# bitlayer-org/tap-stark

Hardware: AMD Instinct MI355X
Metric: trace cells/sec (proofs/sec alongside), 2^20x64 BabyBear trace (higher is better)
Workload: dtype u32

## Files before the change

### tap-stark_amd/csrc/alubench.hip

```cpp
#include "blake3.hpp"
#include "kernels.hpp"
#include "sha256.hpp"

namespace ts {

namespace {

constexpr int BF_ITER = 1024, BF_ILP = 8;
constexpr int B3_ITER = 64;

__global__ void __launch_bounds__(256) k_alu_butterflies(uint32_t* __restrict__ out, uint32_t seed) {
    uint32_t a[BF_ILP], b[BF_ILP];
#pragma unroll
    for (int i = 0; i < BF_ILP; i++) {
        a[i] = (seed + threadIdx.x * 7 + i) % P;
        b[i] = (seed * 3 + threadIdx.x + i) % P;
    }
    const uint32_t w = seed % P;
    for (int it = 0; it < BF_ITER; it++) {
#pragma unroll
        for (int i = 0; i < BF_ILP; i++) {
            const uint32_t x = red2p(a[i]);
            const uint32_t t = mont_mul(b[i], w);
            a[i] = x + t;
            b[i] = x - t + P;
        }
    }
    uint32_t s = 0;
#pragma unroll
    for (int i = 0; i < BF_ILP; i++) s ^= a[i] ^ b[i];
    out[blockIdx.x * blockDim.x + threadIdx.x] = s;
}

__global__ void __launch_bounds__(256) k_alu_blake3(uint32_t* __restrict__ out, uint32_t seed) {
    uint32_t m[16], cv[8];
#pragma unroll
    for (int i = 0; i < 16; i++) m[i] = seed * (i + 1) + threadIdx.x + blockIdx.x * 977;
    for (int it = 0; it < B3_ITER; it++) {
        b3::hash64(m, cv);
#pragma unroll
        for (int i = 0; i < 8; i++) {
            m[i] = cv[i];
            m[8 + i] ^= cv[i];
        }
    }
    uint32_t s = 0;
#pragma unroll
    for (int i = 0; i < 8; i++) s ^= cv[i];
    out[blockIdx.x * blockDim.x + threadIdx.x] = s;
}

constexpr int LDSB_ROUNDS = 256;
template <bool WIDE>
__global__ void __launch_bounds__(256) k_alu_butterflies_lds(uint32_t* __restrict__ out, uint32_t seed) {
    __shared__ uint32_t img[4096 + 128 + 16];
    uint32_t v[16];
#pragma unroll
    for (int i = 0; i < 16; i++) v[i] = (seed + threadIdx.x * 7 + i) % P;
    const uint32_t w = seed % P;
    for (int it = 0; it < LDSB_ROUNDS; it++) {
#pragma unroll
        for (int d = 0; d < 4; d++) {
            const int half = 8 >> d;
#pragma unroll
            for (int q = 0; q < 16; q++)
                if ((q & half) == 0) {
                    const uint32_t x = red2p(v[q]);
                    const uint32_t t = mont_mul(v[q + half], w);
                    v[q] = x + t;
                    v[q + half] = x - t + P;
                }
        }
        if (WIDE) {
            uint4* p4 = reinterpret_cast<uint4*>(img) + threadIdx.x * 4 + (threadIdx.x >> 3);
#pragma unroll
            for (int k = 0; k < 4; k++) p4[k] = make_uint4(v[4 * k], v[4 * k + 1], v[4 * k + 2], v[4 * k + 3]);
            __syncthreads();
            const uint4* r4 = reinterpret_cast<const uint4*>(img) + ((threadIdx.x + 64) & 255) * 4 + (((threadIdx.x + 64) & 255) >> 3);
#pragma unroll
            for (int k = 0; k < 4; k++) {
                const uint4 u = r4[k];
                v[4 * k] = u.x; v[4 * k + 1] = u.y; v[4 * k + 2] = u.z; v[4 * k + 3] = u.w;
            }
        } else {
#pragma unroll
            for (int q = 0; q < 16; q++) {
                const uint32_t i = threadIdx.x + 256u * q;
                img[i + (i >> 5)] = v[q];
            }
            __syncthreads();
#pragma unroll
            for (int q = 0; q < 16; q++) {
                const uint32_t i = 16u * threadIdx.x + q;
                v[q] = img[i + (i >> 5)];
            }
        }
        __syncthreads();
    }
    uint32_t s = 0;
#pragma unroll
    for (int i = 0; i < 16; i++) s ^= v[i];
    out[blockIdx.x * blockDim.x + threadIdx.x] = s;
}

constexpr int SHA_ITER = 32;
__global__ void __launch_bounds__(256) k_alu_sha256(uint32_t* __restrict__ out, uint32_t seed) {
    uint32_t m[16], h[8];
    sha::iv(h);
#pragma unroll
    for (int i = 0; i < 16; i++) m[i] = seed * (i + 1) + threadIdx.x + blockIdx.x * 977;
    for (int it = 0; it < SHA_ITER; it++) {
        sha::compress(h, m);
#pragma unroll
        for (int i = 0; i < 8; i++) m[i] ^= h[i];
    }
    uint32_t s = 0;
#pragma unroll
    for (int i = 0; i < 8; i++) s ^= h[i];
    out[blockIdx.x * blockDim.x + threadIdx.x] = s;
}

}

double alu_ceiling(Context& ctx, int kind) {
    TS_REQUIRE(kind >= 0 && kind <= 4, TS_ERR_INVALID,
               "alu_ceiling: kind is 0 (butterflies), 1 (blake3), 2 (sha256), 3 / 4 (butterflies + LDS round trips)");
    const int blocks = ctx.num_cus * 16, threads = 256, reps = 5;
    DevBuf<uint32_t> out(&ctx, (size_t)blocks * threads);
    hipEvent_t e0, e1;
    TS_HIP(hipEventCreate(&e0));
    TS_HIP(hipEventCreate(&e1));
    auto launch = [&] {
        if (kind == 0)
            hipLaunchKernelGGL(k_alu_butterflies, dim3(blocks), dim3(threads), 0, ctx.stream, out.p, 12345u);
        else if (kind == 1)
            hipLaunchKernelGGL(k_alu_blake3, dim3(blocks), dim3(threads), 0, ctx.stream, out.p, 12345u);
        else if (kind == 3)
            hipLaunchKernelGGL(k_alu_butterflies_lds<false>, dim3(blocks), dim3(threads), 0, ctx.stream, out.p, 12345u);
        else if (kind == 4)
            hipLaunchKernelGGL(k_alu_butterflies_lds<true>, dim3(blocks), dim3(threads), 0, ctx.stream, out.p, 12345u);
        else
            hipLaunchKernelGGL(k_alu_sha256, dim3(blocks), dim3(threads), 0, ctx.stream, out.p, 12345u);
    };
    launch();
    TS_HIP(hipEventRecord(e0, ctx.stream));
    for (int r = 0; r < reps; r++) launch();
    TS_HIP(hipEventRecord(e1, ctx.stream));
    TS_HIP(hipEventSynchronize(e1));
    float ms = 0;
    TS_HIP(hipEventElapsedTime(&ms, e0, e1));
    (void)hipEventDestroy(e0);
    (void)hipEventDestroy(e1);
    const double per = (double)ms / reps * 1e-3;
    const double units = kind == 0 ? (double)BF_ITER * BF_ILP : kind == 1 ? (double)B3_ITER
                         : kind == 2 ? (double)SHA_ITER : (double)LDSB_ROUNDS * 32;
    return units * blocks * threads / per;
}

}
```

### tap-stark_amd/csrc/bb.hpp

```cpp
#pragma once
#include <stdint.h>

#if defined(__HIPCC__)
#include <hip/hip_runtime.h>
#define TS_HD __host__ __device__ __forceinline__
#else
#define TS_HD inline
#endif

namespace ts {

constexpr uint32_t P = 0x78000001u;
constexpr uint32_t P_INV = 0x88000001u;
constexpr uint32_t P_NEG_INV = 0x77ffffffu;
constexpr uint32_t R_MOD_P = 0x0ffffffeu;
constexpr uint32_t R2_MOD_P = 0x45dddde3u;
constexpr uint32_t GENERATOR = 31u;
constexpr uint32_t TWO_ADIC_GEN_27 = 0x1a427a41u;
constexpr uint32_t EF_W = 11u;

TS_HD uint32_t umin32(uint32_t a, uint32_t b) { return a < b ? a : b; }
TS_HD uint32_t add(uint32_t a, uint32_t b) {
    uint32_t s = a + b;
    return umin32(s, s - P);
}
TS_HD uint32_t sub(uint32_t a, uint32_t b) {
    uint32_t d = a - b;
    return umin32(d, d + P);
}
TS_HD uint32_t neg(uint32_t a) { return a ? P - a : 0u; }

TS_HD uint32_t mulhi32(uint32_t a, uint32_t b) {
#if defined(__HIP_DEVICE_COMPILE__)
    return __umulhi(a, b);
#else
    return (uint32_t)(((uint64_t)a * b) >> 32);
#endif
}

TS_HD uint32_t mont_reduce(uint64_t t) {
    uint32_t m = (uint32_t)t * P_NEG_INV;
    uint32_t r = (uint32_t)((t + (uint64_t)m * P) >> 32);
    return umin32(r, r - P);
}
TS_HD uint32_t red2p(uint32_t x) { return umin32(x, x - P); }
TS_HD uint32_t mont_mul_lazy(uint32_t a, uint32_t b) {
    const uint64_t t = (uint64_t)a * b;
    const uint32_t m = (uint32_t)t * P_NEG_INV;
    return (uint32_t)((t + (uint64_t)m * P) >> 32);
}
TS_HD uint32_t mont_mul(uint32_t a, uint32_t b) { return mont_reduce((uint64_t)a * b); }
TS_HD uint32_t to_mont(uint32_t a) { return mont_mul(a, R2_MOD_P); }
TS_HD uint32_t from_mont(uint32_t a) { return mont_reduce((uint64_t)a); }

TS_HD uint32_t mul(uint32_t a, uint32_t b) { return mont_mul(to_mont(a), b); }

TS_HD uint32_t pow_canon(uint32_t a, uint64_t e) {
    uint32_t r = R_MOD_P, am = to_mont(a);
    while (e) {
        if (e & 1) r = mont_mul(r, am);
        am = mont_mul(am, am);
        e >>= 1;
    }
    return from_mont(r);
}
TS_HD uint32_t mont_pow(uint32_t am, uint64_t e) {
    uint32_t r = R_MOD_P;
    while (e) {
        if (e & 1) r = mont_mul(r, am);
        am = mont_mul(am, am);
        e >>= 1;
    }
    return r;
}
TS_HD uint32_t mont_inv(uint32_t a) {
    uint32_t a2 = mont_mul(a, a), a3 = mont_mul(a2, a), a6 = mont_mul(a3, a3);
    uint32_t a7 = mont_mul(a6, a), a14 = mont_mul(a7, a7), a15 = mont_mul(a14, a);
    uint32_t r = a7;
    for (int k = 0; k < 4; k++) r = mont_mul(r, r);
    r = mont_mul(r, a7);
    for (int w = 0; w < 6; w++) {
        for (int k = 0; k < 4; k++) r = mont_mul(r, r);
        r = mont_mul(r, a15);
    }
    return r;
}
TS_HD uint32_t inv_canon(uint32_t a) { return pow_canon(a, P - 2); }
TS_HD uint32_t two_adic_generator(unsigned bits) {
    return pow_canon(TWO_ADIC_GEN_27, 1ull << (27 - bits));
}

struct alignas(16) Ef {
    uint32_t c[4];
};

TS_HD Ef ef_zero() { return Ef{{0, 0, 0, 0}}; }
TS_HD Ef ef_add(Ef a, Ef b) {
    return Ef{{add(a.c[0], b.c[0]), add(a.c[1], b.c[1]), add(a.c[2], b.c[2]), add(a.c[3], b.c[3])}};
}
TS_HD Ef ef_sub(Ef a, Ef b) {
    return Ef{{sub(a.c[0], b.c[0]), sub(a.c[1], b.c[1]), sub(a.c[2], b.c[2]), sub(a.c[3], b.c[3])}};
}
TS_HD Ef ef_neg(Ef a) { return Ef{{neg(a.c[0]), neg(a.c[1]), neg(a.c[2]), neg(a.c[3])}}; }
TS_HD bool ef_eq(Ef a, Ef b) {
    return a.c[0] == b.c[0] && a.c[1] == b.c[1] && a.c[2] == b.c[2] && a.c[3] == b.c[3];
}
TS_HD Ef ef_mul_base(Ef a, uint32_t bm) {
    return Ef{{mont_mul(a.c[0], bm), mont_mul(a.c[1], bm), mont_mul(a.c[2], bm), mont_mul(a.c[3], bm)}};
}
TS_HD uint64_t lazy_mac(uint64_t acc, uint32_t a, uint32_t b) { return acc + (uint64_t)a * b; }
TS_HD uint64_t lazy_fix(uint64_t acc) {
#if defined(__HIP_DEVICE_COMPILE__)
    typedef uint32_t v2u __attribute__((ext_vector_type(2)));
    v2u u = __builtin_bit_cast(v2u, acc);
    u.y = umin32(u.y, u.y - P);
    return __builtin_bit_cast(uint64_t, u);
#else
    uint32_t hi = (uint32_t)(acc >> 32);
    hi = umin32(hi, hi - P);
    return ((uint64_t)hi << 32) | (uint32_t)acc;
#endif
}
TS_HD uint32_t lazy_finish(uint64_t acc) { return mont_reduce(lazy_fix(acc)); }

TS_HD Ef ef_mul(Ef a, Ef b) {
    constexpr uint32_t W_M = (uint32_t)(((uint64_t)EF_W << 32) % P);
    const uint32_t w1 = mont_mul(b.c[1], W_M), w2 = mont_mul(b.c[2], W_M), w3 = mont_mul(b.c[3], W_M);
    const uint32_t a0 = a.c[0], a1 = a.c[1], a2 = a.c[2], a3 = a.c[3];
    const uint64_t r0 = lazy_mac(lazy_mac(lazy_mac(lazy_mac(0, a0, b.c[0]), a1, w3), a2, w2), a3, w1);
    const uint64_t r1 = lazy_mac(lazy_mac(lazy_mac(lazy_mac(0, a0, b.c[1]), a1, b.c[0]), a2, w3), a3, w2);
    const uint64_t r2 = lazy_mac(lazy_mac(lazy_mac(lazy_mac(0, a0, b.c[2]), a1, b.c[1]), a2, b.c[0]), a3, w3);
    const uint64_t r3 = lazy_mac(lazy_mac(lazy_mac(lazy_mac(0, a0, b.c[3]), a1, b.c[2]), a2, b.c[1]), a3, b.c[0]);
    return Ef{{lazy_finish(r0), lazy_finish(r1), lazy_finish(r2), lazy_finish(r3)}};
}
TS_HD Ef ef_to_mont(Ef a) { return Ef{{to_mont(a.c[0]), to_mont(a.c[1]), to_mont(a.c[2]), to_mont(a.c[3])}}; }
TS_HD Ef ef_from_mont(Ef a) {
    return Ef{{from_mont(a.c[0]), from_mont(a.c[1]), from_mont(a.c[2]), from_mont(a.c[3])}};
}
TS_HD Ef ef_one_mont() { return Ef{{R_MOD_P, 0, 0, 0}}; }
TS_HD Ef ef_from_base(uint32_t a) { return Ef{{a, 0, 0, 0}}; }

TS_HD void ef_inv_parts(Ef a, Ef& num, uint32_t& nrm) {
    constexpr uint32_t W_M = (uint32_t)(((uint64_t)EF_W << 32) % P);
    uint32_t a0 = a.c[0], a1 = a.c[1], a2 = a.c[2], a3 = a.c[3];
    uint32_t A2_0 = add(mont_mul(a0, a0), mont_mul(W_M, mont_mul(a2, a2)));
    uint32_t A2_1 = mont_mul(add(a0, a0), a2);
    uint32_t B2_0 = add(mont_mul(a1, a1), mont_mul(W_M, mont_mul(a3, a3)));
    uint32_t B2_1 = mont_mul(add(a1, a1), a3);
    uint32_t c0 = sub(A2_0, mont_mul(W_M, B2_1));
    uint32_t c1 = sub(A2_1, B2_0);
    nrm = sub(mont_mul(c0, c0), mont_mul(W_M, mont_mul(c1, c1)));
    Ef conj = Ef{{a0, neg(a1), a2, neg(a3)}};
    Ef cc = Ef{{c0, 0, neg(c1), 0}};
    num = ef_mul(conj, cc);
}
TS_HD Ef ef_inv(Ef a) {
    Ef num;
    uint32_t nrm;
    ef_inv_parts(a, num, nrm);
    return ef_mul_base(num, mont_inv(nrm));
}
TS_HD Ef ef_pow(Ef am, uint64_t e) {
    Ef r = ef_one_mont();
    while (e) {
        if (e & 1) r = ef_mul(r, am);
        am = ef_mul(am, am);
        e >>= 1;
    }
    return r;
}

TS_HD uint32_t bitrev32(uint32_t x, unsigned bits) {
#if defined(__HIP_DEVICE_COMPILE__)
    return bits ? (__brev(x) >> (32 - bits)) : 0u;
#else
    uint32_t r = 0;
    for (unsigned i = 0; i < bits; i++) r |= ((x >> i) & 1u) << (bits - 1 - i);
    return r;
#endif
}

}
```

### tap-stark_amd/csrc/context.cpp

```cpp
#include <errno.h>
#include <stdio.h>
#include <time.h>
#include <stdlib.h>
#include "context.hpp"

#include <string.h>

#include "kernels.hpp"

namespace ts {

static bool poison_knob(uint32_t* word) {
    const char* e = getenv("TS_POOL_POISON");
    if (!e || !*e) return false;
    char* end = nullptr;
    errno = 0;
    const unsigned long v = strtoul(e, &end, 0);
    TS_REQUIRE(errno == 0 && end != e && *end == 0 && e[0] != '-' && v <= 0xFFFFFFFFul, TS_ERR_INVALID,
               "TS_POOL_POISON is not a 32-bit word (decimal, 0x hex or 0 octal)");
    *word = (uint32_t)v;
    return true;
}

Context::Context(int dev) : device(dev) {
    pool_debug = getenv("TS_POOL_DEBUG") != nullptr;
    poison_on = poison_knob(&poison_word);
    int count = 0;
    hipError_t e = hipGetDeviceCount(&count);
    if (e != hipSuccess || count == 0)
        throw Error(TS_ERR_HIP, "no HIP device available: the tap-stark HIP path has no CPU fallback");
    TS_REQUIRE(dev >= 0 && dev < count, TS_ERR_INVALID, "device index out of range");
    TS_HIP(hipSetDevice(dev));
    hipDeviceProp_t prop;
    TS_HIP(hipGetDeviceProperties(&prop, dev));
    num_cus = prop.multiProcessorCount;
    max_lds_per_block = prop.sharedMemPerBlock;
    arch_name = prop.gcnArchName;
    arch_name = arch_name.substr(0, arch_name.find(':'));
    TS_HIP(hipStreamCreateWithFlags(&stream, hipStreamNonBlocking));
}

Context::~Context() {
    (void)hipSetDevice(device);
    if (stream) (void)hipStreamSynchronize(stream);
    if (d_twiddle_fwd) (void)hipFree(d_twiddle_fwd);
    if (d_twiddle_inv) (void)hipFree(d_twiddle_inv);
    for (auto& t : scale_tables) (void)hipFree(t.d);
    for (auto& t : sel_tables)
        if (t.d) (void)hipFree(t.d);
    if (d_ticket) (void)hipFree(d_ticket);
    for (auto& kv : free_blocks) (void)hipFree(kv.second);
    for (auto& kv : live_blocks) (void)hipFree(kv.first);
    if (h_pinned) (void)hipHostFree(h_pinned);
    if (h_mailbox) (void)hipHostFree(h_mailbox);
    if (h_mailbox_big) (void)hipHostFree(h_mailbox_big);
    if (h_arena) (void)hipHostFree(h_arena);
    if (stream) (void)hipStreamDestroy(stream);
}

static size_t round_block(size_t bytes) {
    if (bytes < 512) return 512;
    if (bytes < (1u << 20)) {
        size_t r = 512;
        while (r < bytes) r <<= 1;
        return r;
    }
    const size_t g = 1u << 20;
    return (bytes + g - 1) / g * g;
}

void* Context::alloc(size_t bytes) {
    const size_t sz = round_block(bytes);
    auto it = free_blocks.find(sz);
    void* p = nullptr;
    if (it != free_blocks.end()) {
        p = it->second;
        free_blocks.erase(it);
    } else {
        TS_HIP(hipSetDevice(device));
        if (pool_debug) {
            struct timespec ts_;
            clock_gettime(CLOCK_MONOTONIC, &ts_);
            fprintf(stderr, "[ts pool %p t=%.3f ms] hipMalloc %zu KiB (reserved %zu MiB)\n", (void*)this,
                    ts_.tv_sec * 1e3 + ts_.tv_nsec * 1e-6, sz >> 10, bytes_reserved >> 20);
        }
        hipError_t e = hipMalloc(&p, sz);
        if (e != hipSuccess) {
            release_cache();
            e = hipMalloc(&p, sz);
        }
        if (e != hipSuccess) {
            (void)hipGetLastError();
            throw Error(TS_ERR_OOM, "device allocation failed");
        }
        bytes_reserved += sz;
    }
    live_blocks[p] = sz;
    if (poison_on) poison(p, sz);
    return p;
}

void Context::poison(void* p, size_t bytes) {
    TS_HIP(hipSetDevice(device));
    TS_HIP(hipMemsetD32Async((hipDeviceptr_t)p, (int)poison_word, bytes / 4, stream));
    TS_HIP(hipStreamSynchronize(stream));
    poison_fills++;
}

void Context::free(void* p) {
    if (!p) return;
    auto it = live_blocks.find(p);
    if (it == live_blocks.end()) return;
    free_blocks.emplace(it->second, p);
    live_blocks.erase(it);
}

void Context::release_cache() {
    if (stream) (void)hipStreamSynchronize(stream);
    for (auto& kv : free_blocks) {
        (void)hipFree(kv.second);
        bytes_reserved -= kv.first;
    }
    free_blocks.clear();
}

uint32_t* Context::ticket() {
    if (!d_ticket) {
        TS_HIP(hipMalloc((void**)&d_ticket, 64 * 17));
        TS_HIP(hipMemsetAsync(d_ticket, 0, 64 * 17, stream));
    }
    return d_ticket;
}

const void* Context::stage(const void* src, size_t bytes) {
    const size_t need = (bytes + 63) & ~(size_t)63;
    if (need > h_arena_bytes / 2) {
        sync();
        if (h_arena) (void)hipHostFree(h_arena);
        h_arena = nullptr;
        size_t sz = 1 << 20;
        while (sz / 2 < need) sz <<= 1;
        TS_HIP(hipHostMalloc((void**)&h_arena, sz, hipHostMallocDefault));
        h_arena_bytes = sz;
        h_arena_off = 0;
    }
    if (h_arena_off + need > h_arena_bytes) {
        sync();
        h_arena_off = 0;
    }
    void* p = h_arena + h_arena_off;
    memcpy(p, src, bytes);
    h_arena_off += need;
    return p;
}

void Context::sync_point(void* host, size_t bytes) {
    if (replay_mode == 2 && replay_pos < replay_log.size() && replay_log[replay_pos].size() == bytes) {
        memcpy(host, replay_log[replay_pos++].data(), bytes);
        return;
    }
    sync();
    if (replay_mode == 1) replay_log.emplace_back((const char*)host, (const char*)host + bytes);
}
void Context::d2h_point(void* host_dst, const void* dev_src, size_t bytes) {
    if (replay_mode == 2 && replay_pos < replay_log.size() && replay_log[replay_pos].size() == bytes) {
        memcpy(host_dst, replay_log[replay_pos++].data(), bytes);
        return;
    }
    if (bytes) TS_HIP(hipMemcpyAsync(host_dst, dev_src, bytes, hipMemcpyDeviceToHost, stream));
    sync();
    if (replay_mode == 1) replay_log.emplace_back((const char*)host_dst, (const char*)host_dst + bytes);
}

uint32_t* Context::mailbox(size_t words) {
    constexpr size_t WORDS = 16384;
    if (words > WORDS / 4) {
        if (words > h_mailbox_big_words) {
            sync();
            if (h_mailbox_big) (void)hipHostFree(h_mailbox_big);
            h_mailbox_big = nullptr;
            h_mailbox_big_words = 0;
            TS_HIP(hipHostMalloc((void**)&h_mailbox_big, words * 4, hipHostMallocDefault));
            h_mailbox_big_words = words;
        }
        return h_mailbox_big;
    }
    if (!h_mailbox) TS_HIP(hipHostMalloc((void**)&h_mailbox, WORDS * 4, hipHostMallocDefault));
    const size_t need = (words + 15) & ~(size_t)15;
    if (mailbox_off + need > WORDS) mailbox_off = 0;
    uint32_t* p = h_mailbox + mailbox_off;
    mailbox_off += need;
    return p;
}

void* Context::pinned(size_t bytes) {
    if (bytes > h_pinned_bytes) {
        if (h_pinned) {
            sync();
            (void)hipHostFree(h_pinned);
        }
        size_t sz = 1 << 16;
        while (sz < bytes) sz <<= 1;
        TS_HIP(hipHostMalloc(&h_pinned, sz, hipHostMallocDefault));
        h_pinned_bytes = sz;
    }
    return h_pinned;
}

std::map<std::string, std::pair<uint64_t, double>> Context::take_kernel_timings() {
    std::map<std::string, std::pair<uint64_t, double>> out;
    sync();
    for (auto& ev : kernel_events) {
        float ms = 0;
        (void)hipEventElapsedTime(&ms, ev.e0, ev.e1);
        auto& slot = out[ev.name];
        slot.first += 1;
        slot.second += ms;
        (void)hipEventDestroy(ev.e0);
        (void)hipEventDestroy(ev.e1);
    }
    kernel_events.clear();
    return out;
}

void Context::ensure_twiddles(unsigned log_size) {
    if (log_size <= twiddle_log && d_twiddle_fwd) return;
    TS_REQUIRE(log_size <= 27, TS_ERR_INVALID, "two-adicity of BabyBear is 27");
    sync();
    if (d_twiddle_fwd) (void)hipFree(d_twiddle_fwd);
    if (d_twiddle_inv) (void)hipFree(d_twiddle_inv);
    d_twiddle_fwd = d_twiddle_inv = nullptr;
    const size_t n = (size_t)1 << log_size;
    TS_HIP(hipMalloc((void**)&d_twiddle_fwd, n * 4));
    TS_HIP(hipMalloc((void**)&d_twiddle_inv, n * 4));
    if (poison_on) {
        poison(d_twiddle_fwd, n * 4);
        poison(d_twiddle_inv, n * 4);
    }
    twiddle_log = log_size;
    launch_build_twiddles(*this, d_twiddle_fwd, d_twiddle_inv, log_size);
}

}
```

### tap-stark_amd/csrc/context.hpp

```cpp
#pragma once
#include <hip/hip_runtime.h>
#include <stdint.h>

#include <map>
#include <stdexcept>
#include <string>
#include <vector>

#include "bb.hpp"

namespace ts {

struct Error : std::runtime_error {
    int code;
    Error(int c, const std::string& m) : std::runtime_error(m), code(c) {}
};

struct FinalPolyNotConstant : Error {
    explicit FinalPolyNotConstant(const std::string& m) : Error(5 , m) {}
};

enum : int {
    TS_OK = 0,
    TS_ERR_INVALID = 1,
    TS_ERR_HIP = 2,
    TS_ERR_OOM = 3,
    TS_ERR_UNSUPPORTED = 4,
    TS_ERR_INVARIANT = 5,
    TS_ERR_BUFFER = 6,
    TS_ERR_COMM = 7,
};

#define TS_HIP(expr)                                                                        \
    do {                                                                                    \
        hipError_t _e = (expr);                                                             \
        if (_e != hipSuccess)                                                               \
            throw ts::Error(ts::TS_ERR_HIP, std::string(#expr) + ": " + hipGetErrorString(_e)); \
    } while (0)

#define TS_REQUIRE(cond, code, msg)                   \
    do {                                              \
        if (!(cond)) throw ts::Error((code), (msg));  \
    } while (0)

struct Context {
    int device = 0;
    hipStream_t stream = nullptr;
    std::string last_error;
    int num_cus = 256;
    size_t max_lds_per_block = 64 * 1024;
    std::string arch_name;

    std::multimap<size_t, void*> free_blocks;
    std::map<void*, size_t> live_blocks;
    size_t bytes_reserved = 0;
    bool pool_debug = false;
    bool poison_on = false;
    uint32_t poison_word = 0;
    uint64_t poison_fills = 0;
    void poison(void* p, size_t bytes);

    uint32_t* d_twiddle_fwd = nullptr;
    uint32_t* d_twiddle_inv = nullptr;
    unsigned twiddle_log = 0;

    struct ScaleTable {
        unsigned log_n, log_blowup;
        uint32_t shift;
        uint32_t* d;
        size_t words;
        uint64_t last_use;
    };
    std::vector<ScaleTable> scale_tables;
    uint64_t scale_clock = 0;
    struct SelTable {
        uint32_t* d = nullptr;
        unsigned log_n = ~0u, log_qd = ~0u;
        uint32_t shift = 0;
        uint64_t last_use = 0;
    };
    SelTable sel_tables[2];
    uint64_t sel_clock = 0;

    uint32_t* d_ticket = nullptr;
    uint32_t* ticket();

    unsigned lde_pass_mask = 7;

    uint32_t* h_mailbox = nullptr;
    size_t mailbox_off = 0;
    uint32_t* h_mailbox_big = nullptr;
    size_t h_mailbox_big_words = 0;
    uint32_t* mailbox(size_t words);

    void* h_pinned = nullptr;
    size_t h_pinned_bytes = 0;
    char* h_arena = nullptr;
    size_t h_arena_bytes = 0, h_arena_off = 0;
    const void* stage(const void* src, size_t bytes);

    bool timing = false;
    std::vector<std::pair<std::string, float>> stage_ms;

    struct KernelEvent {
        const char* name;
        hipEvent_t e0, e1;
    };
    bool kernel_timing = false;
    std::vector<KernelEvent> kernel_events;
    std::map<std::string, std::pair<uint64_t, double>> take_kernel_timings();

    uint64_t pow_hints_accepted = 0, pow_hints_rejected = 0, pow_host_grinds = 0;
    uint64_t local_quotient_fallbacks = 0;

    explicit Context(int dev);
    ~Context();
    Context(const Context&) = delete;

    void* alloc(size_t bytes);
    void free(void* p);
    template <class T>
    T* alloc_n(size_t n) { return static_cast<T*>(alloc(n * sizeof(T))); }
    void release_cache();

    int replay_mode = 0;
    size_t replay_pos = 0;
    std::vector<std::vector<char>> replay_log;
    void sync_point(void* host, size_t bytes);
    void d2h_point(void* host_dst, const void* dev_src, size_t bytes);
    void* pinned(size_t bytes);
    void ensure_twiddles(unsigned log_size);
    void sync() { TS_HIP(hipStreamSynchronize(stream)); }
};

template <class T>
struct DevBuf {
    Context* ctx = nullptr;
    T* p = nullptr;
    size_t n = 0;
    DevBuf() = default;
    DevBuf(Context* c, size_t count) : ctx(c), p(c->alloc_n<T>(count)), n(count) {}
    DevBuf(const DevBuf&) = delete;
    DevBuf& operator=(const DevBuf&) = delete;
    DevBuf(DevBuf&& o) noexcept : ctx(o.ctx), p(o.p), n(o.n) { o.p = nullptr; }
    DevBuf& operator=(DevBuf&& o) noexcept {
        if (this != &o) {
            reset();
            ctx = o.ctx; p = o.p; n = o.n; o.p = nullptr;
        }
        return *this;
    }
    ~DevBuf() { reset(); }
    void reset() {
        if (p) ctx->free(p);
        p = nullptr;
    }
};

struct KernelTimer {
    Context* ctx;
    Context::KernelEvent ev;
    bool on;
    KernelTimer(Context* c, const char* name) : ctx(c), on(c->kernel_timing) {
        if (on) {
            ev.name = name;
            (void)hipEventCreate(&ev.e0);
            (void)hipEventCreate(&ev.e1);
            (void)hipEventRecord(ev.e0, ctx->stream);
        }
    }
    ~KernelTimer() {
        if (on) {
            (void)hipEventRecord(ev.e1, ctx->stream);
            ctx->kernel_events.push_back(ev);
        }
    }
};

#define TS_LAUNCH_NAMED(ctx, name, kernel, grid, block, lds, ...)                   \
    do {                                                                            \
        ts::KernelTimer _kt(&(ctx), name);                                          \
        hipLaunchKernelGGL(kernel, grid, block, lds, (ctx).stream, __VA_ARGS__);    \
    } while (0)
#define TS_LAUNCH(ctx, kernel, ...) TS_LAUNCH_NAMED(ctx, #kernel, kernel, __VA_ARGS__)

struct StageTimer {
    Context* ctx;
    const char* name;
    hipEvent_t e0 = nullptr, e1 = nullptr;
    StageTimer(Context* c, const char* n) : ctx(c), name(n) {
        if (ctx->timing) {
            (void)hipEventCreate(&e0);
            (void)hipEventCreate(&e1);
            (void)hipEventRecord(e0, ctx->stream);
        }
    }
    ~StageTimer() {
        if (ctx->timing && e0) {
            (void)hipEventRecord(e1, ctx->stream);
            (void)hipEventSynchronize(e1);
            float ms = 0;
            (void)hipEventElapsedTime(&ms, e0, e1);
            ctx->stage_ms.emplace_back(name, ms);
            (void)hipEventDestroy(e0);
            (void)hipEventDestroy(e1);
        }
    }
};

}
```

### tap-stark_amd/csrc/kernels.hpp

```cpp
#pragma once
#include <stdint.h>

#include "bb.hpp"
#include "context.hpp"
#include "ntt_plan.hpp"

namespace ts {

struct ColMat {
    uint32_t* d = nullptr;
    uint64_t height = 0;
    uint32_t width = 0;
    uint64_t col_stride = 0;
};

void launch_build_twiddles(Context& ctx, uint32_t* W, uint32_t* Winv, unsigned log_size);
void launch_build_shift_tables(Context& ctx, uint32_t* lo, uint32_t* hi, uint32_t n_hi,
                               uint32_t n_cosets, uint32_t shift_mont, unsigned log_N,
                               unsigned log_blowup, uint32_t scale_mont);
const uint32_t* coset_scale_table(Context& ctx, unsigned log_n, unsigned log_blowup, uint32_t shift);
void launch_transpose_bitrev(Context& ctx, const uint32_t* src, uint32_t* dst, unsigned log_n,
                             uint32_t w, uint64_t dst_col_stride, uint32_t src_width = 0);
bool launch_transpose_bitrev_r16(Context& ctx, const uint32_t* src, uint32_t* dst, unsigned log_n, uint32_t w,
                                 uint64_t dst_col_stride, uint32_t src_width = 0);
void launch_transpose_plain(Context& ctx, const uint32_t* src, uint32_t* dst, uint64_t n, uint32_t w,
                            uint64_t dst_col_stride);
void launch_transpose_to_row_major(Context& ctx, const uint32_t* src, uint64_t col_stride,
                                   uint32_t* dst, uint64_t h, uint32_t w);
void launch_transpose_unbitrev(Context& ctx, const uint32_t* src, uint64_t col_stride, uint32_t* dst,
                               unsigned log_h, uint32_t w);
void coset_lde(Context& ctx, uint32_t* evals, uint64_t in_col_stride, uint32_t ncols, unsigned log_n,
               unsigned log_blowup, uint32_t shift, uint32_t* out, uint64_t out_col_stride,
               uint32_t beta0 = 0, uint32_t n_beta = 0, bool first_round_done = false,
               uint32_t* evals2 = nullptr, uint32_t shift2 = 0, uint32_t gw = 0, bool stage_timers = true);

constexpr uint32_t LDE_NO_OWN = 0xffffffffu;
int lde_own_coset_used(unsigned log_n, unsigned log_blowup, uint32_t shift);

inline void ntt_require_shape(const NttPlan& p, uint32_t ncols, uint64_t stride_a, uint64_t stride_b, bool lde) {
    if (const char* why = ntt_plan_refusal(p, ncols, stride_a, stride_b, lde)) throw Error(TS_ERR_INVALID, why);
}
void launch_contig_inverse(Context& ctx, const NttPlan& p, uint32_t* data, uint64_t col_stride, uint32_t ncols,
                           bool first_round_done = false, uint32_t* data2 = nullptr, uint32_t gw = 0xffffffffu);
void launch_contig_forward(Context& ctx, const NttPlan& p, uint32_t* data, uint64_t col_stride, uint32_t ncols,
                           uint32_t n_blocks, uint32_t gw = 0xffffffffu, uint32_t own_a = LDE_NO_OWN,
                           uint32_t own_b = LDE_NO_OWN);

void dft_columns(Context& ctx, uint32_t* cols, uint64_t col_stride, uint32_t ncols, unsigned log_n, bool inverse,
                 uint32_t shift);
void dft_batch(Context& ctx, const uint32_t* in, uint32_t* out, unsigned log_n, uint32_t w, bool inverse,
               uint32_t shift);
void coset_lde_batch(Context& ctx, const uint32_t* in, uint32_t* out, unsigned log_n, uint32_t w, unsigned added_bits,
                     uint32_t shift, bool bit_reversed);
void launch_bit_reverse_rows(Context& ctx, const uint32_t* src, uint32_t* dst, unsigned log_h, uint32_t w);

constexpr int MAX_BATCH_MATS = 64;
struct LeafMats {
    const uint32_t* d[MAX_BATCH_MATS];
    uint64_t col_stride[MAX_BATCH_MATS];
    uint32_t width[MAX_BATCH_MATS];
    uint8_t row_shift[MAX_BATCH_MATS];
    uint32_t n_mats;
    uint32_t total_width;
    const uint32_t* const* cols;
};
void launch_leaf_hash(Context& ctx, const LeafMats& mats, uint64_t height, uint32_t* digests);
void launch_leaf_hash_ef_pairs(Context& ctx, const uint32_t* vec, uint64_t n_rows, uint32_t* digests);
struct DevChallenger;
bool launch_merkle_levels(Context& ctx, uint32_t* tree, unsigned log_leaves,
                          DevChallenger* ch = nullptr, uint32_t* root_out = nullptr,
                          Ef* beta_out = nullptr);
void launch_merkle_tree_from(Context& ctx, uint32_t* tree, unsigned log_leaves, unsigned first_level,
                             DevChallenger* ch, uint32_t* root_out, Ef* beta_out);
bool leaf_tree_enabled(unsigned log_leaves);
void launch_commit_tree(Context& ctx, const LeafMats& mats, unsigned log_leaves, uint32_t* tree,
                        uint32_t* root_out = nullptr);
void launch_shard_top(Context& ctx, const uint32_t* subroots, uint32_t G, uint32_t* top,
                      DevChallenger* ch, uint32_t* root_out, Ef* beta_out);
void launch_merkle_one_level(Context& ctx, const uint32_t* children, uint32_t* parents,
                             uint64_t n_parents);
void launch_merkle_inject(Context& ctx, uint32_t* nodes, const uint32_t* inj, uint64_t n);
inline uint64_t merkle_level_offset(unsigned log_leaves, unsigned level) {
    uint64_t off = 0;
    for (unsigned l = 0; l < level; l++) off += (uint64_t)1 << (log_leaves - l);
    return off;
}
inline uint64_t merkle_total_digests(unsigned log_leaves) { return ((uint64_t)2 << log_leaves) - 1; }

struct AirProgram;
const uint32_t* selector_table(Context& ctx, unsigned log_n, unsigned log_qd, uint32_t shift);
constexpr int MAX_QUOTIENT_CHUNKS = 64;
struct QuotOut {
    uint32_t* chunk[MAX_QUOTIENT_CHUNKS];
};
void launch_quotient(Context& ctx, const AirProgram& air, const ColMat& trace_lde, unsigned log_n,
                     unsigned log_qd, const uint32_t* d_consts_mont, const uint32_t* d_alpha_pows_mont,
                     const QuotOut& out, uint64_t row_begin = 0, uint64_t row_end = 0,
                     uint32_t shift = GENERATOR, const ColMat* prep_lde = nullptr, const ColMat* aux_lde = nullptr);
void launch_chunk_mix(Context& ctx, uint32_t* const* d_chunk_ptrs, uint32_t qd, uint64_t rows, uint64_t col_stride,
                      const uint32_t* d_mix_mont);

void launch_check_constraints(Context& ctx, const AirProgram& air, const uint32_t* trace_row_major,
                              uint64_t n, const uint32_t* d_consts_mont,
                              unsigned long long* d_violation, const uint32_t* prep_row_major = nullptr,
                              const uint32_t* aux_row_major = nullptr);

void launch_bary_weights(Context& ctx, unsigned log_n, const Ef* points_mont, uint32_t n_points,
                         Ef* out, uint32_t coset_gen = 0);
struct BaryPending {
    DevBuf<uint32_t> partial[4];
    uint32_t* out[4] = {nullptr, nullptr, nullptr, nullptr};
    uint32_t n_blocks[4] = {0, 0, 0, 0}, n_words[4] = {0, 0, 0, 0};
    uint32_t n = 0, capacity = 2;
};
void launch_bary_dots(Context& ctx, const ColMat& m, unsigned log_n, const Ef* weights,
                      uint32_t n_points, Ef* out, BaryPending* pending = nullptr);
void launch_bary_finish(Context& ctx, BaryPending& pending);
struct ReduceArgs {
    Ef z_mont[2];
    Ef off_mont[2];
    Ef rys[2];
    uint32_t n_points;
    uint32_t accumulate;
};
void launch_reduce(Context& ctx, const ColMat& m, unsigned log_h, const uint32_t* d_alpha_pows_mont,
                   const ReduceArgs& args, Ef* ro);
struct FusedReduceArgs {
    Ef z_mont[2];
    Ef off_t[2];
    Ef k0, k1;
    const uint32_t* chunk_w;
    const uint32_t* chunk[MAX_QUOTIENT_CHUNKS];
    uint64_t chunk_stride;
    uint32_t n_chunks;
    uint64_t row0, rows;
};
void launch_reduce_fused(Context& ctx, const ColMat& trace, unsigned log_h,
                         const uint32_t* d_alpha_pows_mont, const FusedReduceArgs& args, Ef* ro,
                         const ColMat* prep = nullptr, const Ef* prep_off_mont = nullptr,
                         const ColMat* aux = nullptr, const Ef* aux_off_mont = nullptr);
void launch_reduce_low(Context& ctx, const ColMat& trace, unsigned log_n, const uint32_t* d_alpha_pows_mont,
                       const FusedReduceArgs& args, const Ef* weights, uint32_t* out);
void launch_ef_interleave(Context& ctx, const uint32_t* cols, uint64_t col_stride, uint64_t rows, Ef* out);

void launch_fri_fold(Context& ctx, const Ef* in, uint64_t h, Ef beta_canonical, Ef* out,
                     uint32_t* next_digests);
void launch_fri_fold_dev(Context& ctx, const Ef* in, uint64_t h, const Ef* d_beta, Ef* out,
                         uint32_t* next_digests, uint64_t h_global = 0, uint64_t row0 = 0);
struct FriRoundLaunch {
    const Ef* prev = nullptr;
    const Ef* d_beta_prev = nullptr;
    Ef* cur = nullptr;
    uint64_t h = 0;
    uint32_t* tree = nullptr;
    DevChallenger* ch = nullptr;
    uint32_t* root_out = nullptr;
    Ef* beta_out = nullptr;
    uint64_t h_global = 0, row0 = 0;
};
void launch_fri_commit_round(Context& ctx, const FriRoundLaunch& r);
constexpr int FRI_TAIL_LOG = 10;
constexpr uint32_t FRI_POW_NONE = 0xffffffffu;
void launch_fri_tail(Context& ctx, const Ef* in, uint32_t L0, uint32_t blowup, DevChallenger* ch,
                     Ef* tail_vecs, uint32_t* tail_trees, uint32_t* roots_out, Ef* betas_out,
                     Ef* final_out, uint32_t pow_bits = 0, uint32_t* pow_out = nullptr,
                     const Ef* beta_in = nullptr);
void launch_vec_add(Context& ctx, Ef* acc, const Ef* other, uint64_t n);
struct FriGatherDesc {
    const uint32_t* vec;
    const uint32_t* tree;
    uint32_t log_leaves;
    uint32_t shift;
    uint64_t out_vals;
    uint64_t out_path;
};
struct RowGatherJob {
    LeafMats mats;
    uint32_t shift;
    uint32_t pad;
    uint64_t out;
};
void launch_gather_queries(Context& ctx, const RowGatherJob* d_rows, uint32_t n_rows, uint32_t max_row_width,
                           const FriGatherDesc* d_descs, uint32_t n_descs, uint32_t max_log_leaves,
                           const uint32_t* d_indices, uint32_t n_idx, uint32_t* out);

double alu_ceiling(Context& ctx, int kind);
double bench_stage(Context& ctx, int stage, unsigned log_n, uint32_t width, unsigned log_blowup, uint32_t reps);

void launch_trace_fibonacci(Context& ctx, uint32_t* out, uint32_t a, uint32_t b, uint64_t n);
void launch_trace_synth_mul(Context& ctx, uint32_t* out, uint64_t n, uint32_t width, uint64_t seed);
void launch_trace_synth_ext(Context& ctx, uint32_t* out, uint64_t n, uint32_t width, uint64_t seed);

enum : uint8_t { COL_U32 = 0, COL_U16 = 1, COL_U8 = 2, COL_MONTY32 = 3, COL_MONTY31 = 4 };
struct IngestPlan {
    bool planar = false;
    uint64_t height = 0;
    uint32_t width = 0;
    uint64_t stride = 0;
    uint64_t bytes = 0;
    int uniform4 = -1;
    std::vector<uint64_t> table;
};
IngestPlan ingest_plan(const uint8_t* kinds, uint32_t n_kinds, bool planar, uint64_t row_stride, uint64_t height,
                       uint32_t width);
void launch_ingest(Context& ctx, const IngestPlan& plan, const uint8_t* src, uint32_t* out);
void launch_scale_words(Context& ctx, const uint32_t* in, uint32_t* out, uint64_t n, uint32_t mult);
uint32_t monty_ingest_factor(uint32_t kind);

}
```

### tap-stark_amd/csrc/ntt.hip

```cpp
#include "kernels.hpp"

namespace ts {

constexpr int SHIFT_LO_BITS = 10;

__global__ void k_build_twiddles(uint32_t* __restrict__ W, uint32_t* __restrict__ Winv,
                                 unsigned log_size) {
    uint32_t idx = blockIdx.x * blockDim.x + threadIdx.x;
    if (idx >= (1u << log_size)) return;
    if (idx == 0) {
        W[0] = R_MOD_P;
        Winv[0] = R_MOD_P;
        return;
    }
    unsigned logm = 31 - __clz(idx);
    uint32_t i = idx - (1u << logm);
    uint32_t g27 = to_mont(TWO_ADIC_GEN_27);
    uint32_t g = mont_pow(g27, 1ull << (27 - (logm + 1)));
    uint32_t e = bitrev32(i, logm);
    uint32_t w = mont_pow(g, e);
    W[idx] = w;
    Winv[idx] = mont_inv(w);
}

void launch_build_twiddles(Context& ctx, uint32_t* W, uint32_t* Winv, unsigned log_size) {
    uint32_t n = 1u << log_size;
    TS_LAUNCH(ctx, k_build_twiddles, dim3((n + 255) / 256), dim3(256), 0, W, Winv, log_size);
    TS_HIP(hipGetLastError());
}

__global__ void k_build_shift_tables(uint32_t* __restrict__ lo, uint32_t* __restrict__ hi,
                                     uint32_t n_hi, uint32_t shift_mont, unsigned log_N,
                                     unsigned log_blowup, uint32_t scale_mont) {
    uint32_t beta = blockIdx.y;
    uint32_t j = blockIdx.x * blockDim.x + threadIdx.x;
    uint32_t n_lo = 1u << SHIFT_LO_BITS;
    if (j >= n_lo + n_hi) return;
    uint32_t g27 = to_mont(TWO_ADIC_GEN_27);
    uint32_t gN = mont_pow(g27, 1ull << (27 - log_N));
    uint32_t s = mont_mul(shift_mont, mont_pow(gN, bitrev32(beta, log_blowup)));
    if (j < n_lo) {
        lo[beta * n_lo + j] = mont_mul(mont_pow(s, j), scale_mont);
    } else {
        uint32_t jj = j - n_lo;
        hi[beta * n_hi + jj] = mont_pow(s, (uint64_t)jj << SHIFT_LO_BITS);
    }
}

void launch_build_shift_tables(Context& ctx, uint32_t* lo, uint32_t* hi, uint32_t n_hi,
                               uint32_t n_cosets, uint32_t shift_mont, unsigned log_N,
                               unsigned log_blowup, uint32_t scale_mont) {
    const uint32_t n_lo = 1u << SHIFT_LO_BITS;
    TS_LAUNCH(ctx, k_build_shift_tables, dim3((n_lo + n_hi + 255) / 256, n_cosets), dim3(256), 0, lo,
              hi, n_hi, shift_mont, log_N, log_blowup, scale_mont);
    TS_HIP(hipGetLastError());
}

__global__ void __launch_bounds__(256)
k_build_scale_table(const uint32_t* __restrict__ lo, const uint32_t* __restrict__ hi, uint32_t n_hi,
                    unsigned log_n, uint32_t* __restrict__ T) {
    const uint32_t beta = blockIdx.y;
    const uint64_t k = (uint64_t)blockIdx.x * blockDim.x + threadIdx.x;
    if (k >= (1ull << log_n)) return;
    const uint32_t n_lo = 1u << SHIFT_LO_BITS;
    T[((uint64_t)beta << log_n) + k] =
        mont_mul(lo[beta * n_lo + (k & (n_lo - 1))], hi[(uint64_t)beta * n_hi + (k >> SHIFT_LO_BITS)]);
}

const uint32_t* coset_scale_table(Context& ctx, unsigned log_n, unsigned log_blowup, uint32_t shift) {
    for (auto& t : ctx.scale_tables)
        if (t.log_n == log_n && t.log_blowup == log_blowup && t.shift == shift) {
            t.last_use = ++ctx.scale_clock;
            return t.d;
        }
    const uint32_t n_cosets = 1u << log_blowup;
    const size_t words = (size_t)n_cosets << log_n;
    size_t total = words * 4;
    for (auto& t : ctx.scale_tables) total += t.words * 4;
    while (!ctx.scale_tables.empty() && (ctx.scale_tables.size() >= 8 || total > (2ull << 30))) {
        size_t victim = 0;
        for (size_t i = 1; i < ctx.scale_tables.size(); i++)
            if (ctx.scale_tables[i].last_use < ctx.scale_tables[victim].last_use) victim = i;
        ctx.sync();
        total -= ctx.scale_tables[victim].words * 4;
        (void)hipFree(ctx.scale_tables[victim].d);
        ctx.scale_tables.erase(ctx.scale_tables.begin() + victim);
    }
    uint32_t* d = nullptr;
    TS_HIP(hipMalloc((void**)&d, words * 4));
    if (ctx.poison_on) ctx.poison(d, words * 4);
    const uint64_t n = 1ull << log_n;
    const uint32_t n_lo = 1u << SHIFT_LO_BITS;
    const uint32_t n_hi = log_n > (unsigned)SHIFT_LO_BITS ? 1u << (log_n - SHIFT_LO_BITS) : 1u;
    DevBuf<uint32_t> lo(&ctx, (size_t)n_cosets * n_lo), hi(&ctx, (size_t)n_cosets * n_hi);
    const uint32_t n_inv_mont = to_mont(inv_canon((uint32_t)(n % P)));
    launch_build_shift_tables(ctx, lo.p, hi.p, n_hi, n_cosets, to_mont(shift), log_n + log_blowup, log_blowup,
                              n_inv_mont);
    TS_LAUNCH(ctx, k_build_scale_table, dim3((unsigned)((n + 255) / 256), n_cosets), dim3(256), 0,
              (const uint32_t*)lo.p, (const uint32_t*)hi.p, n_hi, log_n, d);
    TS_HIP(hipGetLastError());
    ctx.scale_tables.push_back(Context::ScaleTable{log_n, log_blowup, shift, d, words, ++ctx.scale_clock});
    return d;
}

template <bool TO_COLUMNS, bool BITREV>
__global__ void __launch_bounds__(256)
k_transpose_tile(const uint32_t* __restrict__ src, uint32_t* __restrict__ dst, uint64_t h, unsigned log_h,
                 uint32_t w, uint64_t col_stride, uint32_t rm_width) {
    __shared__ uint32_t tile[64][65];
    const uint64_t p0 = (uint64_t)blockIdx.x * 64;
    const uint32_t c0 = blockIdx.y * 64;
    const uint32_t tx = threadIdx.x & 63, ty = threadIdx.x >> 6;
    auto row_of = [&](uint64_t p) -> uint64_t { return BITREV ? bitrev32((uint32_t)p, log_h) : p; };
    if (p0 + 64 <= h && c0 + 64 <= w) {
        const uint64_t rm = row_of(p0) * rm_width + c0 + tx;
        const uint64_t rm_step = BITREV ? (uint64_t)rm_width << (log_h - 6) : rm_width;
        const uint64_t cm = (uint64_t)(c0 + ty) * col_stride + p0 + tx;
        auto rm_at = [&](int k) {
            const uint32_t i = ty + 4 * (uint32_t)k;
            return rm + (uint64_t)(BITREV ? __brev(i) >> 26 : i) * rm_step;
        };
        auto cm_at = [&](int k) { return cm + (uint64_t)(4 * k) * col_stride; };
        uint32_t t[16];
#pragma unroll
        for (int k = 0; k < 16; k++) t[k] = src[TO_COLUMNS ? rm_at(k) : cm_at(k)];
#pragma unroll
        for (int k = 0; k < 16; k++) (TO_COLUMNS ? tile[ty + 4 * k][tx] : tile[tx][ty + 4 * k]) = t[k];
        __syncthreads();
#pragma unroll
        for (int k = 0; k < 16; k++) t[k] = TO_COLUMNS ? tile[tx][ty + 4 * k] : tile[ty + 4 * k][tx];
#pragma unroll
        for (int k = 0; k < 16; k++) dst[TO_COLUMNS ? cm_at(k) : rm_at(k)] = t[k];
        return;
    }
    auto rm_ok = [&](uint32_t j) { return p0 + j < h && c0 + tx < w; };
    auto cm_ok = [&](uint32_t j) { return c0 + j < w && p0 + tx < h; };
    auto rm_at = [&](uint32_t j) { return row_of(p0 + j) * rm_width + c0 + tx; };
    auto cm_at = [&](uint32_t j) { return (uint64_t)(c0 + j) * col_stride + p0 + tx; };
#pragma unroll
    for (int k = 0; k < 16; k++) {
        const uint32_t j = ty + 4 * (uint32_t)k;
        if (TO_COLUMNS ? rm_ok(j) : cm_ok(j)) (TO_COLUMNS ? tile[j][tx] : tile[tx][j]) = src[TO_COLUMNS ? rm_at(j) : cm_at(j)];
    }
    __syncthreads();
#pragma unroll
    for (int k = 0; k < 16; k++) {
        const uint32_t j = ty + 4 * (uint32_t)k;
        if (TO_COLUMNS ? cm_ok(j) : rm_ok(j)) dst[TO_COLUMNS ? cm_at(j) : rm_at(j)] = TO_COLUMNS ? tile[tx][j] : tile[j][tx];
    }
}

template <bool TO_COLUMNS, bool BITREV>
static void launch_transpose_tile(Context& ctx, const char* name, const uint32_t* src, uint32_t* dst, uint64_t h,
                                  unsigned log_h, uint32_t w, uint64_t col_stride, uint32_t rm_width) {
    if (w == 0 || h == 0) return;
    TS_LAUNCH_NAMED(ctx, name, (k_transpose_tile<TO_COLUMNS, BITREV>), dim3((unsigned)((h + 63) / 64), (w + 63) / 64),
                    dim3(256), 0, src, dst, h, log_h, w, col_stride, rm_width);
    TS_HIP(hipGetLastError());
}

void launch_transpose_bitrev(Context& ctx, const uint32_t* src, uint32_t* dst, unsigned log_n,
                             uint32_t w, uint64_t dst_col_stride, uint32_t src_width) {
    launch_transpose_tile<true, true>(ctx, "k_transpose_bitrev", src, dst, 1ull << log_n, log_n, w, dst_col_stride,
                                      src_width ? src_width : w);
}

void launch_transpose_plain(Context& ctx, const uint32_t* src, uint32_t* dst, uint64_t n, uint32_t w,
                            uint64_t dst_col_stride) {
    launch_transpose_tile<true, false>(ctx, "k_transpose_plain", src, dst, n, 0, w, dst_col_stride, w);
}

void launch_transpose_to_row_major(Context& ctx, const uint32_t* src, uint64_t col_stride,
                                   uint32_t* dst, uint64_t h, uint32_t w) {
    launch_transpose_tile<false, false>(ctx, "k_transpose_to_row_major", src, dst, h, 0, w, col_stride, w);
}

void launch_transpose_unbitrev(Context& ctx, const uint32_t* src, uint64_t col_stride, uint32_t* dst,
                               unsigned log_h, uint32_t w) {
    launch_transpose_tile<false, true>(ctx, "k_transpose_unbitrev", src, dst, 1ull << log_h, log_h, w, col_stride, w);
}

}
```

### tap-stark_amd/csrc/ntt_dft.hip

```cpp
#include <algorithm>

#include "ntt_rounds.hpp"

namespace ts {

constexpr int DFT_LO_BITS = 10;

__device__ __forceinline__ uint32_t dft_factor(const uint32_t* __restrict__ lo, const uint32_t* __restrict__ hi,
                                               uint32_t k) {
    return mont_mul(lo[k & ((1u << DFT_LO_BITS) - 1)], hi[k >> DFT_LO_BITS]);
}

template <bool INV, bool SCALE, int PLAN, int TILE = TILE_ELEMS, int NTM = NT_MID>
__global__ void __launch_bounds__(NTM)
k_dft_mid(uint32_t* data, uint64_t col_stride, unsigned log_len, unsigned log_T, unsigned row_shift,
          const uint32_t* __restrict__ W, const uint32_t* __restrict__ f_lo, const uint32_t* __restrict__ f_hi) {
    __shared__ uint32_t s[padded(TILE)];
    constexpr int PER_THREAD = TILE / NTM;
    if (PLAN == 1) {
        log_len = 8;
        log_T = 5;
    }
    const uint32_t j2_0 = blockIdx.x << log_T;
    uint32_t* g = data + (uint64_t)blockIdx.y * col_stride + j2_0;
    const uint32_t total = 1u << (log_len + log_T);
    const uint32_t tmask = (1u << log_T) - 1;
    auto off = [&](uint32_t i) { return ((i >> log_T) << row_shift) + (i & tmask); };
    if constexpr (PLAN == 1) {
        uint32_t t[PER_THREAD];
#pragma unroll
        for (int k = 0; k < PER_THREAD; k++) t[k] = g[off(threadIdx.x + (uint32_t)k * NTM)];
#pragma unroll
        for (int k = 0; k < PER_THREAD; k++) {
            const uint32_t i = threadIdx.x + (uint32_t)k * NTM;
            if (!INV && SCALE) t[k] = mont_mul_lazy(t[k], dft_factor(f_lo, f_hi, off(i) + j2_0));
            s[pad(i)] = t[k];
        }
    } else {
        for (uint32_t i = threadIdx.x; i < total; i += NTM) {
            uint32_t v = g[off(i)];
            if (!INV && SCALE) v = mont_mul_lazy(v, dft_factor(f_lo, f_hi, off(i) + j2_0));
            s[pad(i)] = v;
        }
    }
    __syncthreads();
    if constexpr (PLAN == 1) {
        if (!INV) {
            radix_round<4, false, 9, NTM, true>(s, 13, 0, 0, 0, W);
            radix_round<4, false, 5, NTM>(s, 13, 4, 0, 0, W);
        } else {
            radix_round<4, true, 5, NTM>(s, 13, 4, 0, 0, W);
            radix_round<4, true, 9, NTM, true>(s, 13, 0, 0, 0, W);
        }
    } else {
        if (!INV) tile_forward_rt<NTM>(s, log_len, log_T, 0, 0, W);
        else tile_inverse_rt<NTM>(s, log_len, log_T, 0, 0, W);
    }
    auto finish = [&](uint32_t v, uint32_t i) {
        if (INV) return SCALE ? mont_mul(v, dft_factor(f_lo, f_hi, off(i) + j2_0)) : red2p(v);
        return row_shift != 0 ? v : red2p(v);
    };
    if constexpr (PLAN == 1) {
        uint32_t t[PER_THREAD];
#pragma unroll
        for (int k = 0; k < PER_THREAD; k++) t[k] = s[pad(threadIdx.x + (uint32_t)k * NTM)];
#pragma unroll
        for (int k = 0; k < PER_THREAD; k++) {
            const uint32_t i = threadIdx.x + (uint32_t)k * NTM;
            g[off(i)] = finish(t[k], i);
        }
    } else {
        for (uint32_t i = threadIdx.x; i < total; i += NTM) g[off(i)] = finish(s[pad(i)], i);
    }
}

__global__ void __launch_bounds__(256)
k_bit_reverse_rows(const uint32_t* __restrict__ src, uint32_t* __restrict__ dst, unsigned log_h, uint32_t w) {
    const uint64_t idx = ((uint64_t)blockIdx.y * gridDim.x + blockIdx.x) * 256 + threadIdx.x;
    const uint64_t r = idx / w;
    if (r >> log_h) return;
    const uint32_t c = (uint32_t)(idx - r * w);
    dst[idx] = src[(uint64_t)bitrev32((uint32_t)r, log_h) * w + c];
}

void launch_bit_reverse_rows(Context& ctx, const uint32_t* src, uint32_t* dst, unsigned log_h, uint32_t w) {
    const uint64_t blocks = ((((uint64_t)w) << log_h) + 255) / 256;
    const uint32_t gx = (uint32_t)std::min<uint64_t>(blocks, 1u << 20);
    TS_LAUNCH(ctx, k_bit_reverse_rows, dim3(gx, (uint32_t)((blocks + gx - 1) / gx)), dim3(256), 0, src, dst, log_h, w);
    TS_HIP(hipGetLastError());
}

template <bool INV, bool SCALE>
static void launch_dft_mid_of(Context& ctx, const NttPlan& p, uint32_t* cols, uint64_t col_stride, uint32_t ncols,
                              const uint32_t* f_lo, const uint32_t* f_hi, const char* const (&names)[3]) {
    const uint32_t* W = INV ? ctx.d_twiddle_inv : ctx.d_twiddle_fwd;
    auto launch = [&](auto kernel) {
        TS_LAUNCH_NAMED(ctx, names[(int)p.mid], kernel, dim3(p.tiles, ncols), dim3(NT_MID), 0, cols, col_stride,
                        p.log_len, p.log_T, p.row_shift, W, f_lo, f_hi);
    };
    if (p.mid == NttMid::TILE16384) launch(k_dft_mid<INV, SCALE, 0, 16384>);
    else if (p.mid == NttMid::FIXED256) launch(k_dft_mid<INV, SCALE, 1>);
    else launch(k_dft_mid<INV, SCALE, 0>);
}

static void launch_dft_mid(Context& ctx, const NttPlan& p, uint32_t* cols, uint64_t col_stride, uint32_t ncols,
                           bool inverse, bool scale, const uint32_t* f_lo, const uint32_t* f_hi) {
    if (inverse)
        launch_dft_mid_of<true, true>(ctx, p, cols, col_stride, ncols, f_lo, f_hi,
                                      {"(k_dft_mid<true, true, 0>)", "(k_dft_mid<true, true, 1>)",
                                       "(k_dft_mid<true, true, 0, 16384>)"});
    else if (scale)
        launch_dft_mid_of<false, true>(ctx, p, cols, col_stride, ncols, f_lo, f_hi,
                                       {"(k_dft_mid<false, true, 0>)", "(k_dft_mid<false, true, 1>)",
                                        "(k_dft_mid<false, true, 0, 16384>)"});
    else
        launch_dft_mid_of<false, false>(ctx, p, cols, col_stride, ncols, f_lo, f_hi,
                                        {"(k_dft_mid<false, false, 0>)", "(k_dft_mid<false, false, 1>)",
                                         "(k_dft_mid<false, false, 0, 16384>)"});
}

void dft_columns(Context& ctx, uint32_t* cols, uint64_t col_stride, uint32_t ncols, unsigned log_n, bool inverse,
                 uint32_t shift) {
    if (ncols == 0) return;
    TS_REQUIRE(shift != 0 && shift < P, TS_ERR_INVALID, "dft: the coset shift must be in [1, p)");
    const NttPlan p = ntt_plan(log_n);
    ntt_require_shape(p, ncols, col_stride, 0, false);
    ctx.ensure_twiddles(log_n == 0 ? 1 : log_n);

    const bool scale = inverse || shift != 1;
    DevBuf<uint32_t> lo, hi;
    if (scale) {
        const uint32_t n_hi = log_n > (unsigned)DFT_LO_BITS ? 1u << (log_n - DFT_LO_BITS) : 1u;
        lo = DevBuf<uint32_t>(&ctx, 1u << DFT_LO_BITS);
        hi = DevBuf<uint32_t>(&ctx, n_hi);
        const uint32_t n_inv = inv_canon((uint32_t)((1ull << log_n) % P));
        launch_build_shift_tables(ctx, lo.p, hi.p, n_hi, 1, to_mont(inverse ? inv_canon(shift) : shift), log_n, 0,
                                  inverse ? to_mont(n_inv) : R_MOD_P);
    }
    if (inverse) {
        if (p.two_pass) launch_contig_inverse(ctx, p, cols, col_stride, ncols);
        launch_dft_mid(ctx, p, cols, col_stride, ncols, true, true, lo.p, hi.p);
    } else {
        launch_dft_mid(ctx, p, cols, col_stride, ncols, false, scale, lo.p, hi.p);
        if (p.two_pass) launch_contig_forward(ctx, p, cols, col_stride, ncols, 1);
    }
    TS_HIP(hipGetLastError());
}

void dft_batch(Context& ctx, const uint32_t* in, uint32_t* out, unsigned log_n, uint32_t w, bool inverse,
               uint32_t shift) {
    const uint64_t n = 1ull << log_n;
    DevBuf<uint32_t> cols(&ctx, (size_t)w * n);
    if (inverse) {
        launch_transpose_bitrev(ctx, in, cols.p, log_n, w, n);
        dft_columns(ctx, cols.p, n, w, log_n, true, shift);
        launch_transpose_to_row_major(ctx, cols.p, n, out, n, w);
    } else {
        launch_transpose_plain(ctx, in, cols.p, n, w, n);
        dft_columns(ctx, cols.p, n, w, log_n, false, shift);
        launch_transpose_unbitrev(ctx, cols.p, n, out, log_n, w);
    }
}

void coset_lde_batch(Context& ctx, const uint32_t* in, uint32_t* out, unsigned log_n, uint32_t w, unsigned added_bits,
                     uint32_t shift, bool bit_reversed) {
    const uint64_t n = 1ull << log_n, N = n << added_bits;
    DevBuf<uint32_t> cols(&ctx, (size_t)w * n), lde(&ctx, (size_t)w * N);
    const bool r16 = lde_own_coset_used(log_n, added_bits, shift) < 0 &&
                     launch_transpose_bitrev_r16(ctx, in, cols.p, log_n, w, n);
    if (!r16) launch_transpose_bitrev(ctx, in, cols.p, log_n, w, n);
    coset_lde(ctx, cols.p, n, w, log_n, added_bits, shift, lde.p, N, 0, 0, r16);
    if (bit_reversed) launch_transpose_to_row_major(ctx, lde.p, N, out, N, w);
    else launch_transpose_unbitrev(ctx, lde.p, N, out, log_n + added_bits, w);
}

}
```

### tap-stark_amd/csrc/ntt_lde.hip

```cpp
#include <stdlib.h>

#include <optional>
#include <type_traits>

#include "ntt_rounds.hpp"

namespace ts {

template <int LM, bool SKIP_R16 = false>
__global__ void __launch_bounds__(chunk_threads(LM))
k_intt_contig(uint32_t* __restrict__ data, uint64_t col_stride, unsigned log_n,
              const uint32_t* __restrict__ Winv, uint32_t* __restrict__ data2, uint32_t gw) {
    __shared__ uint32_t s[padded(1 << LM)];
    const uint32_t c = blockIdx.x;
    uint32_t* col = blockIdx.y < gw ? data + (uint64_t)blockIdx.y * col_stride
                                    : data2 + (uint64_t)(blockIdx.y - gw) * col_stride;
    uint32_t* g = col + ((uint64_t)c << LM);
    chunk_load<LM>(s, g);
    chunk_rounds<LM, true, SKIP_R16>(s, log_n - LM, c, Winv);
    chunk_store<LM, false>(s, g);
}

__global__ void __launch_bounds__(256)
k_transpose_bitrev_r16(const uint32_t* __restrict__ src, uint32_t* __restrict__ dst, unsigned log_n,
                       uint32_t w, uint64_t dst_col_stride, uint32_t src_width,
                       const uint32_t* __restrict__ Winv) {
    __shared__ uint32_t tile[64][65];
    const uint32_t p0 = blockIdx.x << 6;
    const uint32_t c0 = blockIdx.y * 64;
    const uint32_t tx = threadIdx.x & 63, ty = threadIdx.x >> 6;
    const uint32_t rb = bitrev32(p0, log_n);
    const uint64_t row_step = (uint64_t)src_width << (log_n - 6);
    uint32_t v[16];
    if (c0 + tx < w) {
        const uint32_t* sp = src + (uint64_t)rb * src_width + c0 + tx;
#pragma unroll
        for (int q = 0; q < 16; q++) v[q] = sp[(uint64_t)(__brev(16 * ty + (uint32_t)q) >> 26) * row_step];
    } else {
#pragma unroll
        for (int q = 0; q < 16; q++) v[q] = 0;
    }
    radix_butterflies<4, true, false>(v, log_n - 4, 0, 0, (p0 >> 4) + ty, Winv);
#pragma unroll
    for (int q = 0; q < 16; q++) tile[16 * ty + q][tx] = v[q];
    __syncthreads();
    uint32_t t[16];
#pragma unroll
    for (int k = 0; k < 16; k++) t[k] = tile[tx][ty + 4 * k];
    uint32_t* dp = dst + (uint64_t)(c0 + ty) * dst_col_stride + p0 + tx;
#pragma unroll
    for (int k = 0; k < 16; k++)
        if (c0 + ty + 4 * k < w) dp[(uint64_t)(4 * k) * dst_col_stride] = t[k];
}

template <int LM, int CPW>
__device__ __forceinline__ void lde_fwd_contig_block(uint32_t* __restrict__ out, uint64_t out_col_stride, unsigned log_n,
                                                     const uint32_t* __restrict__ W, const uint32_t beta) {
    __shared__ uint32_t s[padded(1 << LM)];
    constexpr int NT = chunk_threads(LM);
    constexpr int NV = (1 << LM) / 4 / NT;
    uint32_t* col = out + (uint64_t)blockIdx.y * out_col_stride + ((uint64_t)beta << log_n);
    if constexpr (CPW == 1) {
        const uint32_t c = blockIdx.x;
        uint32_t* o = col + ((uint64_t)c << LM);
        chunk_load<LM>(s, o);
        chunk_rounds<LM, false>(s, log_n - LM, c, W);
        chunk_store<LM, true>(s, o);
    } else {
        const uint32_t c0 = blockIdx.x * CPW;
        uint4 v[NV];
        {
            const uint4* g4 = reinterpret_cast<const uint4*>(col + ((uint64_t)c0 << LM));
#pragma unroll
            for (int k = 0; k < NV; k++) v[k] = g4[threadIdx.x + (uint32_t)k * NT];
        }
#pragma unroll 1
        for (int i = 0; i < CPW; i++) {
            const uint32_t c = c0 + i;
#pragma unroll
            for (int k = 0; k < NV; k++) {
                const uint32_t i4 = threadIdx.x + (uint32_t)k * NT;
                const uint32_t a = 4 * i4 + (i4 >> 3);
                s[a] = v[k].x;
                s[a + 1] = v[k].y;
                s[a + 2] = v[k].z;
                s[a + 3] = v[k].w;
            }
            __syncthreads();
            if (i + 1 < CPW) {
                const uint4* g4 = reinterpret_cast<const uint4*>(col + ((uint64_t)(c + 1) << LM));
#pragma unroll
                for (int k = 0; k < NV; k++) v[k] = g4[threadIdx.x + (uint32_t)k * NT];
            }
            chunk_rounds<LM, false>(s, log_n - LM, c, W);
            chunk_store<LM, true>(s, col + ((uint64_t)c << LM));
            __syncthreads();
        }
    }
}

template <int LM, int CPW = 1>
__global__ void __launch_bounds__(chunk_threads(LM), CPW > 1 ? 4 : 1)
k_lde_fwd_contig(uint32_t* __restrict__ out, uint64_t out_col_stride, unsigned log_n,
                 const uint32_t* __restrict__ W) {
    lde_fwd_contig_block<LM, CPW>(out, out_col_stride, log_n, W, blockIdx.z);
}

template <int LM, int CPW = 1>
__global__ void __launch_bounds__(chunk_threads(LM), CPW > 1 ? 4 : 1)
k_lde_fwd_contig_own(uint32_t* __restrict__ out, uint64_t out_col_stride, unsigned log_n,
                     const uint32_t* __restrict__ W, uint32_t gw, uint32_t own_a, uint32_t own_b) {
    const uint32_t own = blockIdx.y < gw ? own_a : own_b;
    lde_fwd_contig_block<LM, CPW>(out, out_col_stride, log_n, W, blockIdx.z + (blockIdx.z >= own ? 1u : 0u));
}

template <int PLAN, int TILE = TILE_ELEMS, int NTM = NT_MID, int LM = LOG_M, bool OWN = false>
__global__ void __launch_bounds__(NTM)
k_lde_mid(const uint32_t* __restrict__ evals, uint64_t in_col_stride, uint32_t* __restrict__ out,
          uint64_t out_col_stride, unsigned log_n, unsigned log_len, unsigned log_T,
          unsigned row_shift, unsigned beta0, unsigned n_cosets, const uint32_t* __restrict__ W,
          const uint32_t* __restrict__ Winv, const uint32_t* __restrict__ scale_a,
          const uint32_t* __restrict__ evals2, const uint32_t* __restrict__ scale_b, uint32_t gw,
          uint32_t own_a, uint32_t own_b) {
    __shared__ uint32_t s[padded(TILE)];
    constexpr int PER_THREAD = TILE / NTM;
    if (PLAN == 1) {
        log_len = 8;
        log_T = 5;
    }
    const bool remap = PLAN == 0 && log_T < 5 && gridDim.x >= 8;
    uint32_t bx = remap ? (blockIdx.x & 7) * (gridDim.x >> 3) + (blockIdx.x >> 3) : blockIdx.x;
    uint32_t col_id = blockIdx.y;
    if constexpr (PLAN == 1) {
        const uint32_t ncols = gridDim.x >> (LM - 5);
        bx = (blockIdx.x & 31) + 32 * (blockIdx.x / (32 * ncols));
        col_id = (blockIdx.x >> 5) % ncols;
    }
    const uint32_t j2_0 = bx << log_T;
    const uint32_t* g = (col_id < gw ? evals + (uint64_t)col_id * in_col_stride
                                     : evals2 + (uint64_t)(col_id - gw) * in_col_stride) + j2_0;
    const uint32_t* __restrict__ scale = col_id < gw ? scale_a : scale_b;
    const uint32_t own = OWN ? (col_id < gw ? own_a : own_b) : 0xffffffffu;
    const uint32_t total = 1u << (log_len + log_T);
    const uint32_t tmask = (1u << log_T) - 1;
    if constexpr (PLAN == 1) {
        uint32_t t[PER_THREAD];
#pragma unroll
        for (int k = 0; k < PER_THREAD; k++) {
            const uint32_t i = threadIdx.x + (uint32_t)k * NTM;
            t[k] = g[((uint64_t)(i >> log_T) << row_shift) + (i & tmask)];
        }
#pragma unroll
        for (int k = 0; k < PER_THREAD; k++) s[pad(threadIdx.x + (uint32_t)k * NTM)] = t[k];
    } else {
        for (uint32_t i = threadIdx.x; i < total; i += NTM)
            s[pad(i)] = g[((uint64_t)(i >> log_T) << row_shift) + (i & tmask)];
    }
    __syncthreads();
    if (PLAN == 1) {
        radix_round<4, true, 5, NTM>(s, 13, 4, 0, 0, Winv);
    } else {
        tile_inverse_rt<NTM>(s, log_len, log_T, 0, 0, Winv);
    }
    uint32_t coef[PER_THREAD];
#pragma unroll
    for (int k = 0; k < PER_THREAD; k++) {
        const uint32_t i = threadIdx.x + (uint32_t)k * NTM;
        coef[k] = i < total ? s[pad(i)] : 0u;
    }
    constexpr int GP = PER_THREAD / 16;
    if constexpr (PLAN == 1) {
#pragma unroll
        for (int j = 0; j < GP; j++) {
            uint32_t v[16];
#pragma unroll
            for (int q = 0; q < 16; q++) v[q] = coef[j + GP * q];
            radix_butterflies<4, true, true>(v, 0, 0, 0, 0, Winv);
#pragma unroll
            for (int q = 0; q < 16; q++) coef[j + GP * q] = v[q];
        }
    }
    constexpr bool PREFETCH = PLAN == 1;
    uint32_t scv[PREFETCH ? 16 : 1];
    const uint32_t* scp = nullptr;
    if constexpr (PREFETCH) {
        const uint32_t i0 = threadIdx.x;
        scp = scale + ((uint64_t)(i0 >> 5) << LM) + (i0 & 31) + j2_0;
        const uint32_t first = OWN && own == 0 ? 1u : 0u;
#pragma unroll
        for (int q = 0; q < 16; q++)
            scv[q] = (scp + ((uint64_t)(beta0 + first) << log_n))[(uint64_t)q * (NTM >> 5) << LM];
    }
    for (uint32_t bl = 0; bl < n_cosets; bl++) {
        if (OWN && bl == own) continue;
        const uint32_t beta = beta0 + bl;
        const uint32_t* sc = scale + ((uint64_t)beta << log_n);
        __syncthreads();
        if constexpr (PLAN == 1) {
#pragma unroll
            for (int j = 0; j < GP; j++) {
                uint32_t v[16];
#pragma unroll
                for (int q = 0; q < 16; q++) v[q] = mont_mul_lazy(coef[j + GP * q], scv[q]);
                const uint32_t nb = OWN && bl + 1 == own ? bl + 2 : bl + 1;
                if (nb < n_cosets) {
                    const uint32_t* nx = scp + ((uint64_t)(beta0 + nb) << log_n);
#pragma unroll
                    for (int q = 0; q < 16; q++) scv[q] = nx[(uint64_t)q * (NTM >> 5) << LM];
                }
                radix_butterflies<4, false, true>(v, 0, 0, 0, 0, W);
#pragma unroll
                for (int q = 0; q < 16; q++) s[pad(threadIdx.x + (uint32_t)(j + GP * q) * NTM)] = v[q];
            }
            __syncthreads();
            uint32_t* og = out + (uint64_t)col_id * out_col_stride + ((uint64_t)bl << log_n) + j2_0;
            radix_round<4, false, 5, NTM>(s, 13, 4, 0, 0, W);
            uint32_t t[PER_THREAD];
#pragma unroll
            for (int k = 0; k < PER_THREAD; k++) t[k] = s[pad(threadIdx.x + (uint32_t)k * NTM)];
            uint32_t* ot = og + ((uint64_t)(threadIdx.x >> 5) << LM) + (threadIdx.x & 31);
#pragma unroll
            for (int k = 0; k < PER_THREAD; k++) ot[(uint64_t)k * (NTM >> 5) << LM] = t[k];
            continue;
        } else {
#pragma unroll
            for (int k = 0; k < PER_THREAD; k++) {
                const uint32_t i = threadIdx.x + (uint32_t)k * NTM;
                if (i < total) {
                    const uint32_t kk = ((i >> log_T) << row_shift) + (i & tmask) + j2_0;
                    s[pad(i)] = mont_mul_lazy(coef[k], sc[kk]);
                }
            }
            __syncthreads();
            tile_forward_rt<NTM>(s, log_len, log_T, 0, 0, W);
        }
        uint32_t* o = out + (uint64_t)col_id * out_col_stride + ((uint64_t)bl << log_n) + j2_0;
        if (row_shift != 0) {
            for (uint32_t i = threadIdx.x; i < total; i += NTM)
                o[((uint64_t)(i >> log_T) << row_shift) + (i & tmask)] = s[pad(i)];
        } else {
            for (uint32_t i = threadIdx.x; i < total; i += NTM)
                o[((uint64_t)(i >> log_T) << row_shift) + (i & tmask)] = red2p(s[pad(i)]);
        }
    }
}

template <bool VEC>
__global__ void __launch_bounds__(256)
k_lde_own_copy(const uint32_t* __restrict__ evals, uint64_t in_col_stride, uint32_t* __restrict__ out,
               uint64_t out_col_stride, unsigned log_n, const uint32_t* __restrict__ evals2, uint32_t gw,
               uint32_t own_a, uint32_t own_b) {
    const uint32_t col = blockIdx.y;
    const uint32_t* src = col < gw ? evals + (uint64_t)col * in_col_stride
                                   : evals2 + (uint64_t)(col - gw) * in_col_stride;
    uint32_t* dst = out + (uint64_t)col * out_col_stride + ((uint64_t)(col < gw ? own_a : own_b) << log_n);
    if constexpr (VEC) {
        const uint4* s4 = reinterpret_cast<const uint4*>(src) + (uint64_t)blockIdx.x * 1024 + threadIdx.x;
        uint4* d4 = reinterpret_cast<uint4*>(dst) + (uint64_t)blockIdx.x * 1024 + threadIdx.x;
        uint4 v[4];
#pragma unroll
        for (int k = 0; k < 4; k++) v[k] = s4[256 * k];
#pragma unroll
        for (int k = 0; k < 4; k++) d4[256 * k] = v[k];
    } else {
        const uint64_t i = (uint64_t)blockIdx.x * 256 + threadIdx.x;
        if (i < (1ull << log_n)) dst[i] = src[i];
    }
}

constexpr const char* INTT_NAME[3] = {"k_intt_contig<12>", "k_intt_contig<13>", "k_intt_contig<14>"};
constexpr const char* INTT_R16_NAME[3] = {"(k_intt_contig<12, true>)", "(k_intt_contig<13, true>)",
                                          "(k_intt_contig<14, true>)"};
constexpr const char* FWD_NAME[3] = {"k_lde_fwd_contig<12>", "k_lde_fwd_contig<13>", "(k_lde_fwd_contig<14, 4>)"};

template <class F>
static void with_chunk_log(unsigned LM, F&& f) {
    if (LM == 12) f(std::integral_constant<int, 12>{});
    else if (LM == 13) f(std::integral_constant<int, 13>{});
    else f(std::integral_constant<int, 14>{});
}

bool launch_transpose_bitrev_r16(Context& ctx, const uint32_t* src, uint32_t* dst, unsigned log_n, uint32_t w,
                                 uint64_t dst_col_stride, uint32_t src_width) {
    if (w == 0 || !ntt_plan(log_n).fused_first_round) return false;
    ctx.ensure_twiddles(log_n);
    TS_LAUNCH(ctx, k_transpose_bitrev_r16, dim3(1u << (log_n - 6), (w + 63) / 64), dim3(256), 0, src, dst, log_n, w,
              dst_col_stride, src_width ? src_width : w, (const uint32_t*)ctx.d_twiddle_inv);
    TS_HIP(hipGetLastError());
    return true;
}

void launch_contig_inverse(Context& ctx, const NttPlan& p, uint32_t* data, uint64_t col_stride, uint32_t ncols,
                           bool first_round_done, uint32_t* data2, uint32_t gw) {
    const uint32_t* Winv = ctx.d_twiddle_inv;
    with_chunk_log(p.LM, [&](auto lm) {
        constexpr int LM = decltype(lm)::value;
        const dim3 g(p.chunks, ncols), b(chunk_threads(LM));
        if (first_round_done)
            TS_LAUNCH_NAMED(ctx, INTT_R16_NAME[LM - 12], (k_intt_contig<LM, true>), g, b, 0, data, col_stride, p.log_n,
                            Winv, data2, gw);
        else
            TS_LAUNCH_NAMED(ctx, INTT_NAME[LM - 12], k_intt_contig<LM>, g, b, 0, data, col_stride, p.log_n, Winv, data2,
                            gw);
    });
}

static void launch_lde_mid(Context& ctx, const NttPlan& p, const uint32_t* evals, uint64_t in_col_stride,
                           uint32_t* out, uint64_t out_col_stride, uint32_t ncols, uint32_t beta0, uint32_t n_beta,
                           const uint32_t* scale, const uint32_t* evals2, const uint32_t* scale2, uint32_t gw,
                           uint32_t own_a, uint32_t own_b) {
    const uint32_t *W = ctx.d_twiddle_fwd, *Winv = ctx.d_twiddle_inv;
    const dim3 grid(p.tiles, ncols), b(NT_MID);
    const dim3 grid1(p.tiles * ncols);
#define TS_MID_ARGS \
    evals, in_col_stride, out, out_col_stride, p.log_n, p.log_len, p.log_T, p.row_shift, beta0, n_beta, W, Winv, scale, \
        evals2, scale2, gw, own_a, own_b
    if (own_a != LDE_NO_OWN && p.mid == NttMid::FIXED256 && p.LM == 12)
        TS_LAUNCH_NAMED(ctx, "k_lde_mid<1>", (k_lde_mid<1, TILE_ELEMS, NT_MID, 12, true>), grid1, b, 0, TS_MID_ARGS);
    else if (own_a != LDE_NO_OWN && p.mid == NttMid::FIXED256 && p.LM == 13)
        TS_LAUNCH_NAMED(ctx, "(k_lde_mid<1, 8192, 512, 13>)", (k_lde_mid<1, 8192, 512, 13, true>), grid1, b, 0,
                        TS_MID_ARGS);
    else if (own_a != LDE_NO_OWN && p.mid == NttMid::FIXED256)
        TS_LAUNCH_NAMED(ctx, "(k_lde_mid<1, 8192, 512, 14>)", (k_lde_mid<1, 8192, 512, 14, true>), grid1, b, 0,
                        TS_MID_ARGS);
    else if (own_a != LDE_NO_OWN)
        TS_LAUNCH_NAMED(ctx, "k_lde_mid<0>", (k_lde_mid<0, TILE_ELEMS, NT_MID, LOG_M, true>), grid, b, 0, TS_MID_ARGS);
    else if (p.mid == NttMid::TILE16384)
        TS_LAUNCH_NAMED(ctx, "(k_lde_mid<0, 16384>)", (k_lde_mid<0, 16384>), grid, b, 0, TS_MID_ARGS);
    else if (p.mid == NttMid::FIXED256 && p.LM == 12)
        TS_LAUNCH_NAMED(ctx, "k_lde_mid<1>", k_lde_mid<1>, grid1, b, 0, TS_MID_ARGS);
    else if (p.mid == NttMid::FIXED256 && p.LM == 13)
        TS_LAUNCH_NAMED(ctx, "(k_lde_mid<1, 8192, 512, 13>)", (k_lde_mid<1, 8192, 512, 13>), grid1, b, 0, TS_MID_ARGS);
    else if (p.mid == NttMid::FIXED256)
        TS_LAUNCH_NAMED(ctx, "(k_lde_mid<1, 8192, 512, 14>)", (k_lde_mid<1, 8192, 512, 14>), grid1, b, 0, TS_MID_ARGS);
    else
        TS_LAUNCH_NAMED(ctx, "k_lde_mid<0>", k_lde_mid<0>, grid, b, 0, TS_MID_ARGS);
#undef TS_MID_ARGS
}

void launch_contig_forward(Context& ctx, const NttPlan& p, uint32_t* data, uint64_t col_stride, uint32_t ncols,
                           uint32_t n_blocks, uint32_t gw, uint32_t own_a, uint32_t own_b) {
    const uint32_t* W = ctx.d_twiddle_fwd;
    with_chunk_log(p.LM, [&](auto lm) {
        constexpr int LM = decltype(lm)::value;
        constexpr int CPW = LM == 14 ? 4 : 1;
        if (own_a != LDE_NO_OWN)
            TS_LAUNCH_NAMED(ctx, FWD_NAME[LM - 12], (k_lde_fwd_contig_own<LM, CPW>),
                            dim3(p.chunks / CPW, ncols, n_blocks - 1), dim3(chunk_threads(LM)), 0, data, col_stride,
                            p.log_n, W, gw, own_a, own_b);
        else
            TS_LAUNCH_NAMED(ctx, FWD_NAME[LM - 12], (k_lde_fwd_contig<LM, CPW>), dim3(p.chunks / CPW, ncols, n_blocks),
                            dim3(chunk_threads(LM)), 0, data, col_stride, p.log_n, W);
    });
}

int lde_own_coset_used(unsigned log_n, unsigned log_blowup, uint32_t shift) {
    if (const char* e = getenv("TS_LDE_OWN_COSET"); e && *e && atoi(e) == 0) return -1;
    if (log_blowup == 0 || log_n + log_blowup > 27 || ntt_plan(log_n).mid == NttMid::TILE16384) return -1;
    return lde_own_coset(log_n, log_blowup, shift);
}

void coset_lde(Context& ctx, uint32_t* evals, uint64_t in_col_stride, uint32_t ncols, unsigned log_n,
               unsigned log_blowup, uint32_t shift, uint32_t* out, uint64_t out_col_stride,
               uint32_t beta0, uint32_t n_beta, bool first_round_done, uint32_t* evals2, uint32_t shift2,
               uint32_t gw, bool stage_timers) {
    if (ncols == 0) return;
    TS_REQUIRE(evals2 == nullptr || (gw >= 1 && gw < ncols && shift2 != 0), TS_ERR_INVALID,
               "coset_lde: second matrix needs its first column and its shift");
    if (evals2 == nullptr) gw = 0xffffffffu;
    TS_REQUIRE(log_n + log_blowup <= 27, TS_ERR_INVALID, "coset_lde: log_n + log_blowup > 27");
    const NttPlan p = ntt_plan(log_n);
    ntt_require_shape(p, ncols, in_col_stride, out_col_stride, true);
    TS_REQUIRE(!first_round_done || p.fused_first_round, TS_ERR_INVARIANT,
               "coset_lde: no contiguous inverse pass at this size");
    ctx.ensure_twiddles(log_n == 0 ? 1 : log_n);

    const uint32_t n_cosets = 1u << log_blowup;
    if (n_beta == 0) n_beta = n_cosets - beta0;
    TS_REQUIRE(beta0 < n_cosets && n_beta <= n_cosets - beta0, TS_ERR_INVALID, "coset_lde: coset range");
    const uint32_t* scale = coset_scale_table(ctx, log_n, log_blowup, shift);
    const uint32_t* scale2 = evals2 ? coset_scale_table(ctx, log_n, log_blowup, shift2) : nullptr;

    uint32_t own_a = LDE_NO_OWN, own_b = LDE_NO_OWN;
    if (beta0 == 0 && n_beta == n_cosets && !first_round_done && ctx.lde_pass_mask == 7u) {
        const int a = lde_own_coset_used(log_n, log_blowup, shift);
        const int b = evals2 ? lde_own_coset_used(log_n, log_blowup, shift2) : a;
        if (a >= 0 && b >= 0) {
            own_a = (uint32_t)a;
            own_b = (uint32_t)b;
            const uint64_t n = 1ull << log_n;
            if (p.two_pass)
                TS_LAUNCH_NAMED(ctx, "k_lde_own_copy", k_lde_own_copy<true>, dim3((unsigned)(n >> 12), ncols), dim3(256), 0,
                                (const uint32_t*)evals, in_col_stride, out, out_col_stride, log_n,
                                (const uint32_t*)evals2, gw, own_a, own_b);
            else
                TS_LAUNCH_NAMED(ctx, "k_lde_own_copy", k_lde_own_copy<false>, dim3((unsigned)((n + 255) / 256), ncols),
                                dim3(256), 0, (const uint32_t*)evals, in_col_stride, out, out_col_stride, log_n,
                                (const uint32_t*)evals2, gw, own_a, own_b);
        }
    }

    if (!p.two_pass) {
        launch_lde_mid(ctx, p, evals, in_col_stride, out, out_col_stride, ncols, beta0, n_beta, scale, evals2, scale2,
                       gw, own_a, own_b);
    } else {
        if (ctx.lde_pass_mask & 1u) {
            std::optional<StageTimer> t;
            if (stage_timers) t.emplace(&ctx, "lde: inverse NTT, contiguous stages");
            launch_contig_inverse(ctx, p, evals, in_col_stride, ncols, first_round_done, evals2, gw);
        }
        std::optional<StageTimer> t_rest;
        if (stage_timers) t_rest.emplace(&ctx, "lde: strided pass + forward NTT of the owned cosets");
        if (ctx.lde_pass_mask & 2u)
            launch_lde_mid(ctx, p, evals, in_col_stride, out, out_col_stride, ncols, beta0, n_beta, scale, evals2,
                           scale2, gw, own_a, own_b);
        if (ctx.lde_pass_mask & 4u) launch_contig_forward(ctx, p, out, out_col_stride, ncols, n_beta, gw, own_a, own_b);
    }
    TS_HIP(hipGetLastError());
}

}
```

### tap-stark_amd/csrc/ntt_rounds.hpp

```cpp
#pragma once
#include "kernels.hpp"
#include "ntt_plan.hpp"

namespace ts {

constexpr int NT_MID = 512;
constexpr int chunk_threads(int lm) { return lm == 14 ? 512 : 256; }

__device__ __forceinline__ uint32_t pad(uint32_t i) { return i + (i >> 5); }
constexpr int padded(int n) { return n + (n >> 5); }

template <int K, bool INV, bool TOP>
__device__ __forceinline__ void radix_butterflies(uint32_t (&v)[1 << K], unsigned s_base, unsigned u0,
                                                  uint32_t c, uint32_t hi,
                                                  const uint32_t* __restrict__ W) {
    constexpr int R = 1 << K;
    if (!INV) {
#pragma unroll
        for (int d = 0; d < K; d++) {
            const int half = R >> (d + 1);
            const uint32_t* __restrict__ wp = W + ((1u << (s_base + u0 + d)) + (c << (u0 + d)) + (hi << d));
#pragma unroll
            for (int q = 0; q < R; q++) {
                if ((q & half) == 0) {
                    const uint32_t a = red2p(v[q]);
                    uint32_t t = v[q + half];
                    if (TOP && (q >> (K - d)) == 0) t = red2p(t);
                    else t = mont_mul(t, wp[q >> (K - d)]);
                    v[q] = a + t;
                    v[q + half] = a - t + P;
                }
            }
        }
    } else {
#pragma unroll
        for (int d = K - 1; d >= 0; d--) {
            const int half = R >> (d + 1);
            const uint32_t* __restrict__ wp = W + ((1u << (s_base + u0 + d)) + (c << (u0 + d)) + (hi << d));
#pragma unroll
            for (int q = 0; q < R; q++) {
                if ((q & half) == 0) {
                    const uint32_t a = red2p(v[q]), b = red2p(v[q + half]);
                    v[q] = a + b;
                    uint32_t dlt = a - b + P;
                    if (!(TOP && (q >> (K - d)) == 0)) dlt = mont_mul_lazy(dlt, wp[q >> (K - d)]);
                    v[q + half] = dlt;
                }
            }
        }
    }
}

template <int K, bool INV, int LOG_DL, int NTH, bool TOP = false>
__device__ __forceinline__ void radix_round(uint32_t* s, unsigned log_total, unsigned u0,
                                            unsigned s_base, uint32_t c,
                                            const uint32_t* __restrict__ W) {
    constexpr int R = 1 << K;
    const unsigned log_dl = LOG_DL >= 0 ? (unsigned)LOG_DL : log_total - u0 - K;
    const uint32_t n_groups = 1u << (log_total - K);
    for (uint32_t g0 = threadIdx.x; g0 < n_groups; g0 += NTH) {
        uint32_t g = g0;
        if (LOG_DL == 4 && K < 5) {
            constexpr uint32_t B = 9 - K;
            const uint32_t x = ((g >> 4) ^ (g >> B)) & 1u;
            g ^= (x << 4) | (x << B);
        }
        const uint32_t lo = g & ((1u << log_dl) - 1);
        const uint32_t hi = g >> log_dl;
        const uint32_t base = (hi << (K + log_dl)) + lo;
        const uint32_t pbase = pad(base);
        uint32_t addr[R];
#pragma unroll
        for (int q = 0; q < R; q++) {
            if (LOG_DL >= 5)
                addr[q] = pbase + (uint32_t)q * ((1u << (LOG_DL >= 5 ? LOG_DL : 5)) +
                                                 (1u << (LOG_DL >= 5 ? LOG_DL - 5 : 0)));
            else if (LOG_DL == 4)
                addr[q] = pbase + 16u * (uint32_t)q + ((uint32_t)q >> 1);
            else if (LOG_DL == 0 && K == 4)
                addr[q] = pbase + (uint32_t)q;
            else
                addr[q] = pad(base + ((uint32_t)q << log_dl));
        }
        uint32_t v[R];
#pragma unroll
        for (int q = 0; q < R; q++) v[q] = s[addr[q]];
        radix_butterflies<K, INV, TOP>(v, s_base, u0, c, hi, W);
#pragma unroll
        for (int q = 0; q < R; q++) s[addr[q]] = v[q];
    }
    __syncthreads();
}

template <bool INV, int NTH>
__device__ __forceinline__ void radix_round_rt(int k, uint32_t* s, unsigned log_total, unsigned u0,
                                               unsigned s_base, uint32_t c,
                                               const uint32_t* __restrict__ W) {
    switch (k) {
        case 4: radix_round<4, INV, -1, NTH>(s, log_total, u0, s_base, c, W); break;
        case 3: radix_round<3, INV, -1, NTH>(s, log_total, u0, s_base, c, W); break;
        case 2: radix_round<2, INV, -1, NTH>(s, log_total, u0, s_base, c, W); break;
        default: radix_round<1, INV, -1, NTH>(s, log_total, u0, s_base, c, W); break;
    }
}

template <int NTH>
__device__ __forceinline__ void tile_forward_rt(uint32_t* s, unsigned log_len, unsigned log_T,
                                                unsigned s_base, uint32_t c,
                                                const uint32_t* __restrict__ W) {
    if (log_len == 0) return;
    const unsigned nr = (log_len + 3) / 4, q = log_len / nr, rem = log_len % nr;
    unsigned u = 0;
    for (unsigned r = 0; r < nr; r++) {
        const unsigned k = q + (r < rem ? 1u : 0u);
        radix_round_rt<false, NTH>((int)k, s, log_len + log_T, u, s_base, c, W);
        u += k;
    }
}
template <int NTH>
__device__ __forceinline__ void tile_inverse_rt(uint32_t* s, unsigned log_len, unsigned log_T,
                                                unsigned s_base, uint32_t c,
                                                const uint32_t* __restrict__ Winv) {
    if (log_len == 0) return;
    const unsigned nr = (log_len + 3) / 4, q = log_len / nr, rem = log_len % nr;
    unsigned u = log_len;
    for (int r = (int)nr - 1; r >= 0; r--) {
        const unsigned k = q + ((unsigned)r < rem ? 1u : 0u);
        u -= k;
        radix_round_rt<true, NTH>((int)k, s, log_len + log_T, u, s_base, c, Winv);
    }
}

template <int LM>
__device__ __forceinline__ void chunk_load(uint32_t* s, const uint32_t* __restrict__ g) {
    constexpr int NT = chunk_threads(LM);
    const uint4* g4 = reinterpret_cast<const uint4*>(g);
    uint4 v[(1 << LM) / 4 / NT];
#pragma unroll
    for (int k = 0; k < (1 << LM) / 4 / NT; k++) v[k] = g4[threadIdx.x + (uint32_t)k * NT];
#pragma unroll
    for (int k = 0; k < (1 << LM) / 4 / NT; k++) {
        const uint32_t i4 = threadIdx.x + (uint32_t)k * NT;
        const uint32_t a = 4 * i4 + (i4 >> 3);
        s[a] = v[k].x;
        s[a + 1] = v[k].y;
        s[a + 2] = v[k].z;
        s[a + 3] = v[k].w;
    }
    __syncthreads();
}
template <int LM, bool CANON>
__device__ __forceinline__ void chunk_store(const uint32_t* s, uint32_t* __restrict__ g) {
    constexpr int NT = chunk_threads(LM);
    uint4* g4 = reinterpret_cast<uint4*>(g);
#pragma unroll
    for (int k = 0; k < (1 << LM) / 4 / NT; k++) {
        const uint32_t i4 = threadIdx.x + (uint32_t)k * NT;
        const uint32_t a = 4 * i4 + (i4 >> 3);
        if (CANON)
            g4[i4] = make_uint4(red2p(s[a]), red2p(s[a + 1]), red2p(s[a + 2]), red2p(s[a + 3]));
        else
            g4[i4] = make_uint4(s[a], s[a + 1], s[a + 2], s[a + 3]);
    }
}

template <int LM, bool INV, bool SKIP_R16 = false>
__device__ __forceinline__ void chunk_rounds(uint32_t* s, unsigned sb, uint32_t c, const uint32_t* __restrict__ W) {
    constexpr int NT = chunk_threads(LM);
    constexpr int K0 = LM == 12 ? 4 : 5;
    constexpr int K1 = LM == 14 ? 5 : 4;
    static_assert(K0 + K1 + 4 == LM, "chunk plan");
    if (!INV) {
        radix_round<K0, false, LM - K0, NT>(s, LM, 0, sb, c, W);
        radix_round<K1, false, 4, NT>(s, LM, K0, sb, c, W);
        radix_round<4, false, 0, NT>(s, LM, K0 + K1, sb, c, W);
    } else {
        if (!SKIP_R16) radix_round<4, true, 0, NT>(s, LM, K0 + K1, sb, c, W);
        radix_round<K1, true, 4, NT>(s, LM, K0, sb, c, W);
        radix_round<K0, true, LM - K0, NT>(s, LM, 0, sb, c, W);
    }
}

}
```

### tap-stark_amd/probe/field_probe.hip

```cpp
#include <stdio.h>
#include <string.h>

#include <vector>

#include "bb.hpp"
#include "ntt_rounds.hpp"

using namespace ts;

namespace {

constexpr uint32_t MAGIC = 0x42465042u;

enum Op : uint32_t {
    OP_CONSTS = 0,
    OP_ADD = 1,
    OP_SUB = 2,
    OP_NEG = 3,
    OP_RED2P = 4,
    OP_MONT_REDUCE = 5,
    OP_MONT_MUL = 6,
    OP_TO_MONT = 7,
    OP_FROM_MONT = 8,
    OP_MUL = 9,
    OP_MONT_INV = 10,
    OP_INV_CANON = 11,
    OP_MONT_MUL_LAZY = 12,
    OP_LAZY = 13,
    OP_EF_ADD = 14,
    OP_EF_SUB = 15,
    OP_EF_NEG = 16,
    OP_EF_MUL = 17,
    OP_EF_MUL_BASE = 18,
    OP_EF_INV_PARTS = 19,
    OP_EF_INV = 20,
    OP_EF_POW = 21,
    OP_BITREV = 22,
    OP_TWO_ADIC_GEN = 23,
    OP_POW_CANON = 24,
    OP_MONT_POW = 25,
    N_SCALAR_OPS = 26,
    OP_BFLY = 32,
    OP_BFLY_END = 36,
};

struct Shape {
    uint32_t n_in, n_out;
};
TS_HD Shape shape_of(uint32_t op) {
    switch (op) {
        case OP_CONSTS: return {1, 8};
        case OP_ADD: case OP_SUB: case OP_MONT_REDUCE: case OP_MONT_MUL: case OP_MUL: case OP_MONT_MUL_LAZY:
        case OP_BITREV: return {2, 1};
        case OP_NEG: case OP_RED2P: case OP_TO_MONT: case OP_FROM_MONT: case OP_MONT_INV: case OP_INV_CANON:
        case OP_TWO_ADIC_GEN: return {1, 1};
        case OP_LAZY: return {20, 3};
        case OP_EF_ADD: case OP_EF_SUB: case OP_EF_MUL: return {8, 4};
        case OP_EF_NEG: case OP_EF_INV: return {4, 4};
        case OP_EF_MUL_BASE: return {5, 4};
        case OP_EF_INV_PARTS: return {4, 5};
        case OP_EF_POW: return {6, 4};
        case OP_POW_CANON: case OP_MONT_POW: return {3, 1};
        default: return (op >= OP_BFLY && op < OP_BFLY_END) ? Shape{32, 16} : Shape{0, 0};
    }
}

TS_HD Ef ef_at(const uint32_t* p) { return Ef{{p[0], p[1], p[2], p[3]}}; }
TS_HD void ef_put(uint32_t* p, Ef e) {
    for (int k = 0; k < 4; k++) p[k] = e.c[k];
}
TS_HD uint64_t u64_at(const uint32_t* p) { return (uint64_t)p[0] | ((uint64_t)p[1] << 32); }

TS_HD void apply(uint32_t op, const uint32_t* in, uint32_t* out) {
    switch (op) {
        case OP_CONSTS:
            out[0] = P; out[1] = P_INV; out[2] = P_NEG_INV; out[3] = R_MOD_P; out[4] = R2_MOD_P;
            out[5] = GENERATOR; out[6] = TWO_ADIC_GEN_27; out[7] = EF_W;
            break;
        case OP_ADD: out[0] = add(in[0], in[1]); break;
        case OP_SUB: out[0] = sub(in[0], in[1]); break;
        case OP_NEG: out[0] = neg(in[0]); break;
        case OP_RED2P: out[0] = red2p(in[0]); break;
        case OP_MONT_REDUCE: out[0] = mont_reduce(u64_at(in)); break;
        case OP_MONT_MUL: out[0] = mont_mul(in[0], in[1]); break;
        case OP_TO_MONT: out[0] = to_mont(in[0]); break;
        case OP_FROM_MONT: out[0] = from_mont(in[0]); break;
        case OP_MUL: out[0] = mul(in[0], in[1]); break;
        case OP_MONT_INV: out[0] = mont_inv(in[0]); break;
        case OP_INV_CANON: out[0] = inv_canon(in[0]); break;
        case OP_MONT_MUL_LAZY: out[0] = mont_mul_lazy(in[0], in[1]); break;
        case OP_LAZY: {
            uint64_t acc = u64_at(in);
            const uint32_t n = in[2] < 8 ? in[2] : 8, mask = in[3];
            for (uint32_t i = 0; i < n; i++) {
                acc = lazy_mac(acc, in[4 + 2 * i], in[5 + 2 * i]);
                if ((mask >> i) & 1u) acc = lazy_fix(acc);
            }
            out[0] = (uint32_t)acc;
            out[1] = (uint32_t)(acc >> 32);
            out[2] = lazy_finish(acc);
            break;
        }
        case OP_EF_ADD: ef_put(out, ef_add(ef_at(in), ef_at(in + 4))); break;
        case OP_EF_SUB: ef_put(out, ef_sub(ef_at(in), ef_at(in + 4))); break;
        case OP_EF_NEG: ef_put(out, ef_neg(ef_at(in))); break;
        case OP_EF_MUL: ef_put(out, ef_mul(ef_at(in), ef_at(in + 4))); break;
        case OP_EF_MUL_BASE: ef_put(out, ef_mul_base(ef_at(in), in[4])); break;
        case OP_EF_INV_PARTS: {
            Ef num;
            uint32_t nrm;
            ef_inv_parts(ef_at(in), num, nrm);
            ef_put(out, num);
            out[4] = nrm;
            break;
        }
        case OP_EF_INV: ef_put(out, ef_inv(ef_at(in))); break;
        case OP_EF_POW: ef_put(out, ef_pow(ef_at(in), u64_at(in + 4))); break;
        case OP_BITREV: out[0] = bitrev32(in[0], in[1]); break;
        case OP_TWO_ADIC_GEN: out[0] = two_adic_generator(in[0]); break;
        case OP_POW_CANON: out[0] = pow_canon(in[0], u64_at(in + 1)); break;
        case OP_MONT_POW: out[0] = mont_pow(in[0], u64_at(in + 1)); break;
        default: break;
    }
}

__global__ void __launch_bounds__(256) k_probe(uint32_t op, const uint32_t* __restrict__ in, uint32_t* __restrict__ out,
                                               uint32_t count, uint32_t n_in, uint32_t n_out) {
    const uint32_t i = blockIdx.x * 256u + threadIdx.x;
    if (i >= count) return;
    apply(op, in + (size_t)i * n_in, out + (size_t)i * n_out);
}

template <bool INV, bool TOP>
__global__ void __launch_bounds__(256) k_probe_bfly(const uint32_t* __restrict__ in, uint32_t* __restrict__ out,
                                                    uint32_t count) {
    const uint32_t i = blockIdx.x * 256u + threadIdx.x;
    if (i >= count) return;
    uint32_t v[16];
    for (int q = 0; q < 16; q++) v[q] = in[(size_t)i * 32 + q];
    radix_butterflies<4, INV, TOP>(v, 0, 0, 0, 0, in + (size_t)i * 32 + 16);
    for (int q = 0; q < 16; q++) out[(size_t)i * 16 + q] = v[q];
}

bool read_words(const char* path, std::vector<uint32_t>& w) {
    FILE* f = fopen(path, "rb");
    if (!f) return false;
    fseek(f, 0, SEEK_END);
    const long sz = ftell(f);
    fseek(f, 0, SEEK_SET);
    if (sz < 0 || sz % 4) {
        fclose(f);
        return false;
    }
    w.resize((size_t)sz / 4);
    const bool ok = fread(w.data(), 4, w.size(), f) == w.size();
    fclose(f);
    return ok;
}

#define HIP_OR_FAIL(call)                                                                      \
    do {                                                                                       \
        hipError_t e_ = (call);                                                                \
        if (e_ != hipSuccess) {                                                                \
            fprintf(stderr, "field_probe: %s: %s\n", #call, hipGetErrorString(e_));            \
            return 4;                                                                          \
        }                                                                                      \
    } while (0)

int run_device(uint32_t op, const uint32_t* in, uint32_t* out, uint32_t count, Shape sh) {
    uint32_t *d_in = nullptr, *d_out = nullptr;
    const size_t in_bytes = (size_t)count * sh.n_in * 4, out_bytes = (size_t)count * sh.n_out * 4;
    HIP_OR_FAIL(hipMalloc(&d_in, in_bytes));
    HIP_OR_FAIL(hipMalloc(&d_out, out_bytes));
    HIP_OR_FAIL(hipMemcpy(d_in, in, in_bytes, hipMemcpyHostToDevice));
    HIP_OR_FAIL(hipMemset(d_out, 0xff, out_bytes));
    const dim3 grid((count + 255) / 256), block(256);
    switch (op) {
        case OP_BFLY + 0: k_probe_bfly<false, false><<<grid, block>>>(d_in, d_out, count); break;
        case OP_BFLY + 1: k_probe_bfly<true, false><<<grid, block>>>(d_in, d_out, count); break;
        case OP_BFLY + 2: k_probe_bfly<false, true><<<grid, block>>>(d_in, d_out, count); break;
        case OP_BFLY + 3: k_probe_bfly<true, true><<<grid, block>>>(d_in, d_out, count); break;
        default: k_probe<<<grid, block>>>(op, d_in, d_out, count, sh.n_in, sh.n_out); break;
    }
    HIP_OR_FAIL(hipGetLastError());
    HIP_OR_FAIL(hipDeviceSynchronize());
    HIP_OR_FAIL(hipMemcpy(out, d_out, out_bytes, hipMemcpyDeviceToHost));
    HIP_OR_FAIL(hipFree(d_in));
    HIP_OR_FAIL(hipFree(d_out));
    return 0;
}

}

int main(int argc, char** argv) {
    bool host = false;
    const char* paths[2] = {nullptr, nullptr};
    int n_paths = 0;
    for (int i = 1; i < argc; i++) {
        if (!strcmp(argv[i], "--host")) host = true;
        else if (n_paths < 2) paths[n_paths++] = argv[i];
        else n_paths = 3;
    }
    if (n_paths != 2) {
        fprintf(stderr, "usage: field_probe [--host] <operands> <results>\n");
        return 2;
    }
    std::vector<uint32_t> in;
    if (!read_words(paths[0], in) || in.size() < 2 || in[0] != MAGIC) {
        fprintf(stderr, "field_probe: cannot read operand file %s\n", paths[0]);
        return 2;
    }
    if (!host) {
        int n_dev = 0;
        if (hipGetDeviceCount(&n_dev) != hipSuccess || n_dev < 1) {
            fprintf(stderr, "field_probe: no HIP device (use --host for the host build of the primitives)\n");
            return 3;
        }
        HIP_OR_FAIL(hipSetDevice(0));
    }
    std::vector<uint32_t> res{MAGIC, in[1]};
    size_t pos = 2;
    for (uint32_t r = 0; r < in[1]; r++) {
        if (pos + 4 > in.size()) {
            fprintf(stderr, "field_probe: record %u: truncated header\n", r);
            return 2;
        }
        const uint32_t op = in[pos], count = in[pos + 1];
        const Shape sh = shape_of(op);
        if (sh.n_in == 0 || in[pos + 2] != sh.n_in || in[pos + 3] != sh.n_out || count == 0 ||
            (size_t)count * sh.n_in > in.size() - (pos + 4)) {
            fprintf(stderr, "field_probe: record %u: op %u with %u x (%u -> %u) words is malformed\n", r, op, count,
                    in[pos + 2], in[pos + 3]);
            return 2;
        }
        if (host && op >= N_SCALAR_OPS) {
            fprintf(stderr, "field_probe: record %u: op %u exists in the device build only\n", r, op);
            return 2;
        }
        const uint32_t* src = &in[pos + 4];
        res.insert(res.end(), {op, count, sh.n_out});
        const size_t at = res.size();
        res.resize(at + (size_t)count * sh.n_out, 0xffffffffu);
        if (host) {
            for (uint32_t i = 0; i < count; i++) apply(op, src + (size_t)i * sh.n_in, &res[at + (size_t)i * sh.n_out]);
        } else if (int rc = run_device(op, src, &res[at], count, sh)) {
            return rc;
        }
        pos += 4 + (size_t)count * sh.n_in;
    }
    FILE* f = fopen(paths[1], "wb");
    if (!f || fwrite(res.data(), 4, res.size(), f) != res.size() || fclose(f) != 0) {
        fprintf(stderr, "field_probe: cannot write %s\n", paths[1]);
        return 2;
    }
    return 0;
}
```

Before: 25.48 billion.

## Use Plantard multiplication with precomputed 64-bit twiddles in NTT kernels

Adds Plantard modular multiplication for BabyBear, which uses twiddles precomputed as 64-bit constants stored in new uint2 tables. Most NTT/LDE kernels (inverse contiguous, transpose-bitrev, mid tiles, some forward ones) now template on the twiddle type and use Plantard butterflies. This aims to cut the multiply and reduce instruction count per butterfly compared with Montgomery. In exchange, twiddle tables double in memory traffic and the lazy-reduction structure of inverse butterflies changes. It also adds a microbenchmark and probe ops.

```diff
diff --git a/tap-stark_amd/csrc/alubench.hip b/tap-stark_amd/csrc/alubench.hip
--- a/tap-stark_amd/csrc/alubench.hip
+++ b/tap-stark_amd/csrc/alubench.hip
@@ -22,6 +22,30 @@
         for (int i = 0; i < BF_ILP; i++) {
             const uint32_t x = red2p(a[i]);
             const uint32_t t = mont_mul(b[i], w);
+            a[i] = x + t;
+            b[i] = x - t + P;
+        }
+    }
+    uint32_t s = 0;
+#pragma unroll
+    for (int i = 0; i < BF_ILP; i++) s ^= a[i] ^ b[i];
+    out[blockIdx.x * blockDim.x + threadIdx.x] = s;
+}
+
+__global__ void __launch_bounds__(256) k_alu_butterflies_plant(uint32_t* __restrict__ out, uint32_t seed) {
+    uint32_t a[BF_ILP], b[BF_ILP];
+#pragma unroll
+    for (int i = 0; i < BF_ILP; i++) {
+        a[i] = (seed + threadIdx.x * 7 + i) % P;
+        b[i] = (seed * 3 + threadIdx.x + i) % P;
+    }
+    const uint64_t w = plant_const(seed % P);
+    const uint32_t w_lo = (uint32_t)w, w_hi = (uint32_t)(w >> 32);
+    for (int it = 0; it < BF_ITER; it++) {
+#pragma unroll
+        for (int i = 0; i < BF_ILP; i++) {
+            const uint32_t x = red2p(a[i]);
+            const uint32_t t = plant_mul(b[i], w_lo, w_hi);
             a[i] = x + t;
             b[i] = x - t + P;
         }
@@ -123,8 +147,9 @@
 }
 
 double alu_ceiling(Context& ctx, int kind) {
-    TS_REQUIRE(kind >= 0 && kind <= 4, TS_ERR_INVALID,
-               "alu_ceiling: kind is 0 (butterflies), 1 (blake3), 2 (sha256), 3 / 4 (butterflies + LDS round trips)");
+    TS_REQUIRE(kind >= 0 && kind <= 5, TS_ERR_INVALID,
+               "alu_ceiling: kind is 0 (butterflies), 1 (blake3), 2 (sha256), 3 / 4 (butterflies + LDS round trips), "
+               "5 (Plantard butterflies)");
     const int blocks = ctx.num_cus * 16, threads = 256, reps = 5;
     DevBuf<uint32_t> out(&ctx, (size_t)blocks * threads);
     hipEvent_t e0, e1;
@@ -139,6 +164,8 @@
             hipLaunchKernelGGL(k_alu_butterflies_lds<false>, dim3(blocks), dim3(threads), 0, ctx.stream, out.p, 12345u);
         else if (kind == 4)
             hipLaunchKernelGGL(k_alu_butterflies_lds<true>, dim3(blocks), dim3(threads), 0, ctx.stream, out.p, 12345u);
+        else if (kind == 5)
+            hipLaunchKernelGGL(k_alu_butterflies_plant, dim3(blocks), dim3(threads), 0, ctx.stream, out.p, 12345u);
         else
             hipLaunchKernelGGL(k_alu_sha256, dim3(blocks), dim3(threads), 0, ctx.stream, out.p, 12345u);
     };
@@ -152,7 +179,7 @@
     (void)hipEventDestroy(e0);
     (void)hipEventDestroy(e1);
     const double per = (double)ms / reps * 1e-3;
-    const double units = kind == 0 ? (double)BF_ITER * BF_ILP : kind == 1 ? (double)B3_ITER
+    const double units = kind == 0 || kind == 5 ? (double)BF_ITER * BF_ILP : kind == 1 ? (double)B3_ITER
                          : kind == 2 ? (double)SHA_ITER : (double)LDSB_ROUNDS * 32;
     return units * blocks * threads / per;
 }
diff --git a/tap-stark_amd/csrc/bb.hpp b/tap-stark_amd/csrc/bb.hpp
--- a/tap-stark_amd/csrc/bb.hpp
+++ b/tap-stark_amd/csrc/bb.hpp
@@ -54,6 +54,16 @@
 TS_HD uint32_t from_mont(uint32_t a) { return mont_reduce((uint64_t)a); }
 
 TS_HD uint32_t mul(uint32_t a, uint32_t b) { return mont_mul(to_mont(a), b); }
+
+constexpr uint64_t P_INV64 = 0x383FFFFF88000001ull;
+TS_HD uint64_t plant_const(uint32_t w_canonical) {
+    return (uint64_t)mont_mul(to_mont(w_canonical), P - R2_MOD_P) * P_INV64;
+}
+TS_HD uint32_t plant_mul(uint32_t a, uint32_t w_lo, uint32_t w_hi) {
+    const uint32_t u = (uint32_t)((uint64_t)a * w_hi + mulhi32(a, w_lo));
+    return (uint32_t)(((uint64_t)u * P + P) >> 32);
+}
+TS_HD uint32_t plant_mul(uint32_t a, uint64_t wp) { return plant_mul(a, (uint32_t)wp, (uint32_t)(wp >> 32)); }
 
 TS_HD uint32_t pow_canon(uint32_t a, uint64_t e) {
     uint32_t r = R_MOD_P, am = to_mont(a);
diff --git a/tap-stark_amd/csrc/context.cpp b/tap-stark_amd/csrc/context.cpp
--- a/tap-stark_amd/csrc/context.cpp
+++ b/tap-stark_amd/csrc/context.cpp
@@ -45,6 +45,8 @@
     if (stream) (void)hipStreamSynchronize(stream);
     if (d_twiddle_fwd) (void)hipFree(d_twiddle_fwd);
     if (d_twiddle_inv) (void)hipFree(d_twiddle_inv);
+    if (d_plant_fwd) (void)hipFree(d_plant_fwd);
+    if (d_plant_inv) (void)hipFree(d_plant_inv);
     for (auto& t : scale_tables) (void)hipFree(t.d);
     for (auto& t : sel_tables)
         if (t.d) (void)hipFree(t.d);
@@ -241,4 +243,22 @@
     launch_build_twiddles(*this, d_twiddle_fwd, d_twiddle_inv, log_size);
 }
 
-}
+void Context::ensure_plant_twiddles(unsigned log_size) {
+    if (log_size <= plant_log && d_plant_fwd) return;
+    TS_REQUIRE(log_size <= 27, TS_ERR_INVALID, "two-adicity of BabyBear is 27");
+    sync();
+    if (d_plant_fwd) (void)hipFree(d_plant_fwd);
+    if (d_plant_inv) (void)hipFree(d_plant_inv);
+    d_plant_fwd = d_plant_inv = nullptr;
+    const size_t n = (size_t)1 << log_size;
+    TS_HIP(hipMalloc((void**)&d_plant_fwd, n * 8));
+    TS_HIP(hipMalloc((void**)&d_plant_inv, n * 8));
+    if (poison_on) {
+        poison(d_plant_fwd, n * 8);
+        poison(d_plant_inv, n * 8);
+    }
+    plant_log = log_size;
+    launch_build_plant_twiddles(*this, d_plant_fwd, d_plant_inv, log_size);
+}
+
+}
diff --git a/tap-stark_amd/csrc/context.hpp b/tap-stark_amd/csrc/context.hpp
--- a/tap-stark_amd/csrc/context.hpp
+++ b/tap-stark_amd/csrc/context.hpp
@@ -63,6 +63,9 @@
     uint32_t* d_twiddle_fwd = nullptr;
     uint32_t* d_twiddle_inv = nullptr;
     unsigned twiddle_log = 0;
+    uint2* d_plant_fwd = nullptr;
+    uint2* d_plant_inv = nullptr;
+    unsigned plant_log = 0;
 
     struct ScaleTable {
         unsigned log_n, log_blowup;
@@ -130,6 +133,7 @@
     void d2h_point(void* host_dst, const void* dev_src, size_t bytes);
     void* pinned(size_t bytes);
     void ensure_twiddles(unsigned log_size);
+    void ensure_plant_twiddles(unsigned log_size);
     void sync() { TS_HIP(hipStreamSynchronize(stream)); }
 };
 
diff --git a/tap-stark_amd/csrc/kernels.hpp b/tap-stark_amd/csrc/kernels.hpp
--- a/tap-stark_amd/csrc/kernels.hpp
+++ b/tap-stark_amd/csrc/kernels.hpp
@@ -15,6 +15,7 @@
 };
 
 void launch_build_twiddles(Context& ctx, uint32_t* W, uint32_t* Winv, unsigned log_size);
+void launch_build_plant_twiddles(Context& ctx, uint2* WP, uint2* WPinv, unsigned log_size);
 void launch_build_shift_tables(Context& ctx, uint32_t* lo, uint32_t* hi, uint32_t n_hi,
                                uint32_t n_cosets, uint32_t shift_mont, unsigned log_N,
                                unsigned log_blowup, uint32_t scale_mont);
diff --git a/tap-stark_amd/csrc/ntt.hip b/tap-stark_amd/csrc/ntt.hip
--- a/tap-stark_amd/csrc/ntt.hip
+++ b/tap-stark_amd/csrc/ntt.hip
@@ -4,28 +4,43 @@
 
 constexpr int SHIFT_LO_BITS = 10;
 
-__global__ void k_build_twiddles(uint32_t* __restrict__ W, uint32_t* __restrict__ Winv,
-                                 unsigned log_size) {
-    uint32_t idx = blockIdx.x * blockDim.x + threadIdx.x;
-    if (idx >= (1u << log_size)) return;
-    if (idx == 0) {
-        W[0] = R_MOD_P;
-        Winv[0] = R_MOD_P;
-        return;
-    }
+__device__ __forceinline__ uint32_t twiddle_mont(uint32_t idx) {
+    if (idx == 0) return R_MOD_P;
     unsigned logm = 31 - __clz(idx);
     uint32_t i = idx - (1u << logm);
     uint32_t g27 = to_mont(TWO_ADIC_GEN_27);
     uint32_t g = mont_pow(g27, 1ull << (27 - (logm + 1)));
     uint32_t e = bitrev32(i, logm);
-    uint32_t w = mont_pow(g, e);
+    return mont_pow(g, e);
+}
+
+__global__ void k_build_twiddles(uint32_t* __restrict__ W, uint32_t* __restrict__ Winv,
+                                 unsigned log_size) {
+    uint32_t idx = blockIdx.x * blockDim.x + threadIdx.x;
+    if (idx >= (1u << log_size)) return;
+    const uint32_t w = twiddle_mont(idx);
     W[idx] = w;
     Winv[idx] = mont_inv(w);
+}
+
+__global__ void k_build_plant_twiddles(uint2* __restrict__ WP, uint2* __restrict__ WPinv, unsigned log_size) {
+    uint32_t idx = blockIdx.x * blockDim.x + threadIdx.x;
+    if (idx >= (1u << log_size)) return;
+    const uint32_t w = twiddle_mont(idx);
+    const uint64_t f = plant_const(from_mont(w)), b = plant_const(from_mont(mont_inv(w)));
+    WP[idx] = make_uint2((uint32_t)f, (uint32_t)(f >> 32));
+    WPinv[idx] = make_uint2((uint32_t)b, (uint32_t)(b >> 32));
 }
 
 void launch_build_twiddles(Context& ctx, uint32_t* W, uint32_t* Winv, unsigned log_size) {
     uint32_t n = 1u << log_size;
     TS_LAUNCH(ctx, k_build_twiddles, dim3((n + 255) / 256), dim3(256), 0, W, Winv, log_size);
+    TS_HIP(hipGetLastError());
+}
+
+void launch_build_plant_twiddles(Context& ctx, uint2* WP, uint2* WPinv, unsigned log_size) {
+    uint32_t n = 1u << log_size;
+    TS_LAUNCH(ctx, k_build_plant_twiddles, dim3((n + 255) / 256), dim3(256), 0, WP, WPinv, log_size);
     TS_HIP(hipGetLastError());
 }
 
diff --git a/tap-stark_amd/csrc/ntt_dft.hip b/tap-stark_amd/csrc/ntt_dft.hip
--- a/tap-stark_amd/csrc/ntt_dft.hip
+++ b/tap-stark_amd/csrc/ntt_dft.hip
@@ -11,10 +11,10 @@
     return mont_mul(lo[k & ((1u << DFT_LO_BITS) - 1)], hi[k >> DFT_LO_BITS]);
 }
 
-template <bool INV, bool SCALE, int PLAN, int TILE = TILE_ELEMS, int NTM = NT_MID>
+template <bool INV, bool SCALE, int PLAN, int TILE = TILE_ELEMS, int NTM = NT_MID, class TW = uint32_t>
 __global__ void __launch_bounds__(NTM)
 k_dft_mid(uint32_t* data, uint64_t col_stride, unsigned log_len, unsigned log_T, unsigned row_shift,
-          const uint32_t* __restrict__ W, const uint32_t* __restrict__ f_lo, const uint32_t* __restrict__ f_hi) {
+          const TW* __restrict__ W, const uint32_t* __restrict__ f_lo, const uint32_t* __restrict__ f_hi) {
     __shared__ uint32_t s[padded(TILE)];
     constexpr int PER_THREAD = TILE / NTM;
     if (PLAN == 1) {
@@ -90,17 +90,25 @@
     TS_HIP(hipGetLastError());
 }
 
+template <bool INV, int PLAN, int TILE> struct DftMidFormOf {
+    using type = uint2;
+};
+template <> struct DftMidFormOf<true, 0, TILE_ELEMS> {
+    using type = uint32_t;
+};
+template <bool INV, int PLAN, int TILE> using DftMidForm = typename DftMidFormOf<INV, PLAN, TILE>::type;
+
 template <bool INV, bool SCALE>
 static void launch_dft_mid_of(Context& ctx, const NttPlan& p, uint32_t* cols, uint64_t col_stride, uint32_t ncols,
                               const uint32_t* f_lo, const uint32_t* f_hi, const char* const (&names)[3]) {
-    const uint32_t* W = INV ? ctx.d_twiddle_inv : ctx.d_twiddle_fwd;
+    const TwTables W = INV ? twiddles_inv(ctx) : twiddles_fwd(ctx);
     auto launch = [&](auto kernel) {
         TS_LAUNCH_NAMED(ctx, names[(int)p.mid], kernel, dim3(p.tiles, ncols), dim3(NT_MID), 0, cols, col_stride,
                         p.log_len, p.log_T, p.row_shift, W, f_lo, f_hi);
     };
-    if (p.mid == NttMid::TILE16384) launch(k_dft_mid<INV, SCALE, 0, 16384>);
-    else if (p.mid == NttMid::FIXED256) launch(k_dft_mid<INV, SCALE, 1>);
-    else launch(k_dft_mid<INV, SCALE, 0>);
+    if (p.mid == NttMid::TILE16384) launch(k_dft_mid<INV, SCALE, 0, 16384, NT_MID, DftMidForm<INV, 0, 16384>>);
+    else if (p.mid == NttMid::FIXED256) launch(k_dft_mid<INV, SCALE, 1, TILE_ELEMS, NT_MID, DftMidForm<INV, 1, TILE_ELEMS>>);
+    else launch(k_dft_mid<INV, SCALE, 0, TILE_ELEMS, NT_MID, DftMidForm<INV, 0, TILE_ELEMS>>);
 }
 
 static void launch_dft_mid(Context& ctx, const NttPlan& p, uint32_t* cols, uint64_t col_stride, uint32_t ncols,
@@ -126,6 +134,7 @@
     const NttPlan p = ntt_plan(log_n);
     ntt_require_shape(p, ncols, col_stride, 0, false);
     ctx.ensure_twiddles(log_n == 0 ? 1 : log_n);
+    ctx.ensure_plant_twiddles(log_n == 0 ? 1 : log_n);
 
     const bool scale = inverse || shift != 1;
     DevBuf<uint32_t> lo, hi;
diff --git a/tap-stark_amd/csrc/ntt_lde.hip b/tap-stark_amd/csrc/ntt_lde.hip
--- a/tap-stark_amd/csrc/ntt_lde.hip
+++ b/tap-stark_amd/csrc/ntt_lde.hip
@@ -7,10 +7,10 @@
 
 namespace ts {
 
-template <int LM, bool SKIP_R16 = false>
+template <int LM, bool SKIP_R16 = false, class TW = uint32_t>
 __global__ void __launch_bounds__(chunk_threads(LM))
 k_intt_contig(uint32_t* __restrict__ data, uint64_t col_stride, unsigned log_n,
-              const uint32_t* __restrict__ Winv, uint32_t* __restrict__ data2, uint32_t gw) {
+              const TW* __restrict__ Winv, uint32_t* __restrict__ data2, uint32_t gw) {
     __shared__ uint32_t s[padded(1 << LM)];
     const uint32_t c = blockIdx.x;
     uint32_t* col = blockIdx.y < gw ? data + (uint64_t)blockIdx.y * col_stride
@@ -24,7 +24,7 @@
 __global__ void __launch_bounds__(256)
 k_transpose_bitrev_r16(const uint32_t* __restrict__ src, uint32_t* __restrict__ dst, unsigned log_n,
                        uint32_t w, uint64_t dst_col_stride, uint32_t src_width,
-                       const uint32_t* __restrict__ Winv) {
+                       const uint2* __restrict__ Winv) {
     __shared__ uint32_t tile[64][65];
     const uint32_t p0 = blockIdx.x << 6;
     const uint32_t c0 = blockIdx.y * 64;
@@ -53,9 +53,9 @@
         if (c0 + ty + 4 * k < w) dp[(uint64_t)(4 * k) * dst_col_stride] = t[k];
 }
 
-template <int LM, int CPW>
+template <int LM, int CPW, class TW>
 __device__ __forceinline__ void lde_fwd_contig_block(uint32_t* __restrict__ out, uint64_t out_col_stride, unsigned log_n,
-                                                     const uint32_t* __restrict__ W, const uint32_t beta) {
+                                                     const TW* __restrict__ W, const uint32_t beta) {
     __shared__ uint32_t s[padded(1 << LM)];
     constexpr int NT = chunk_threads(LM);
     constexpr int NV = (1 << LM) / 4 / NT;
@@ -99,27 +99,28 @@
     }
 }
 
-template <int LM, int CPW = 1>
+template <int LM, int CPW = 1, class TW = uint32_t>
 __global__ void __launch_bounds__(chunk_threads(LM), CPW > 1 ? 4 : 1)
 k_lde_fwd_contig(uint32_t* __restrict__ out, uint64_t out_col_stride, unsigned log_n,
-                 const uint32_t* __restrict__ W) {
+                 const TW* __restrict__ W) {
     lde_fwd_contig_block<LM, CPW>(out, out_col_stride, log_n, W, blockIdx.z);
 }
 
-template <int LM, int CPW = 1>
+template <int LM, int CPW = 1, class TW = uint32_t>
 __global__ void __launch_bounds__(chunk_threads(LM), CPW > 1 ? 4 : 1)
 k_lde_fwd_contig_own(uint32_t* __restrict__ out, uint64_t out_col_stride, unsigned log_n,
-                     const uint32_t* __restrict__ W, uint32_t gw, uint32_t own_a, uint32_t own_b) {
+                     const TW* __restrict__ W, uint32_t gw, uint32_t own_a, uint32_t own_b) {
     const uint32_t own = blockIdx.y < gw ? own_a : own_b;
     lde_fwd_contig_block<LM, CPW>(out, out_col_stride, log_n, W, blockIdx.z + (blockIdx.z >= own ? 1u : 0u));
 }
 
-template <int PLAN, int TILE = TILE_ELEMS, int NTM = NT_MID, int LM = LOG_M, bool OWN = false>
+template <int PLAN, int TILE = TILE_ELEMS, int NTM = NT_MID, int LM = LOG_M, bool OWN = false, class TWF = uint32_t,
+          class TWI = uint32_t>
 __global__ void __launch_bounds__(NTM)
 k_lde_mid(const uint32_t* __restrict__ evals, uint64_t in_col_stride, uint32_t* __restrict__ out,
           uint64_t out_col_stride, unsigned log_n, unsigned log_len, unsigned log_T,
-          unsigned row_shift, unsigned beta0, unsigned n_cosets, const uint32_t* __restrict__ W,
-          const uint32_t* __restrict__ Winv, const uint32_t* __restrict__ scale_a,
+          unsigned row_shift, unsigned beta0, unsigned n_cosets, const TWF* __restrict__ W,
+          const TWI* __restrict__ Winv, const uint32_t* __restrict__ scale_a,
           const uint32_t* __restrict__ evals2, const uint32_t* __restrict__ scale_b, uint32_t gw,
           uint32_t own_a, uint32_t own_b) {
     __shared__ uint32_t s[padded(TILE)];
@@ -273,6 +274,27 @@
                                           "(k_intt_contig<14, true>)"};
 constexpr const char* FWD_NAME[3] = {"k_lde_fwd_contig<12>", "k_lde_fwd_contig<13>", "(k_lde_fwd_contig<14, 4>)"};
 
+template <int LM> struct ContigForm {
+    using Inv = uint2;
+    using Fwd = uint2;
+};
+template <> struct ContigForm<14> {
+    using Inv = uint2;
+    using Fwd = uint32_t;
+};
+template <int PLAN, int TILE> struct MidForm {
+    using Inv = uint2;
+    using Fwd = uint2;
+};
+template <> struct MidForm<0, TILE_ELEMS> {
+    using Inv = uint2;
+    using Fwd = uint32_t;
+};
+static_assert(std::is_same<ContigForm<12>::Inv, uint2>::value && std::is_same<ContigForm<13>::Inv, uint2>::value &&
+                  std::is_same<ContigForm<14>::Inv, uint2>::value,
+              "the strided inverse rounds (here and in ntt_dft.hip) take canonical words: a Montgomery k_intt_contig "
+              "would have to be reduced on load");
+
 template <class F>
 static void with_chunk_log(unsigned LM, F&& f) {
     if (LM == 12) f(std::integral_constant<int, 12>{});
@@ -283,25 +305,26 @@
 bool launch_transpose_bitrev_r16(Context& ctx, const uint32_t* src, uint32_t* dst, unsigned log_n, uint32_t w,
                                  uint64_t dst_col_stride, uint32_t src_width) {
     if (w == 0 || !ntt_plan(log_n).fused_first_round) return false;
-    ctx.ensure_twiddles(log_n);
+    ctx.ensure_plant_twiddles(log_n);
     TS_LAUNCH(ctx, k_transpose_bitrev_r16, dim3(1u << (log_n - 6), (w + 63) / 64), dim3(256), 0, src, dst, log_n, w,
-              dst_col_stride, src_width ? src_width : w, (const uint32_t*)ctx.d_twiddle_inv);
+              dst_col_stride, src_width ? src_width : w, (const uint2*)ctx.d_plant_inv);
     TS_HIP(hipGetLastError());
     return true;
 }
 
 void launch_contig_inverse(Context& ctx, const NttPlan& p, uint32_t* data, uint64_t col_stride, uint32_t ncols,
                            bool first_round_done, uint32_t* data2, uint32_t gw) {
-    const uint32_t* Winv = ctx.d_twiddle_inv;
+    const TwTables Winv = twiddles_inv(ctx);
     with_chunk_log(p.LM, [&](auto lm) {
         constexpr int LM = decltype(lm)::value;
+        using TW = typename ContigForm<LM>::Inv;
         const dim3 g(p.chunks, ncols), b(chunk_threads(LM));
         if (first_round_done)
-            TS_LAUNCH_NAMED(ctx, INTT_R16_NAME[LM - 12], (k_intt_contig<LM, true>), g, b, 0, data, col_stride, p.log_n,
+            TS_LAUNCH_NAMED(ctx, INTT_R16_NAME[LM - 12], (k_intt_contig<LM, true, TW>), g, b, 0, data, col_stride,
+                            p.log_n, Winv, data2, gw);
+        else
+            TS_LAUNCH_NAMED(ctx, INTT_NAME[LM - 12], (k_intt_contig<LM, false, TW>), g, b, 0, data, col_stride, p.log_n,
                             Winv, data2, gw);
-        else
-            TS_LAUNCH_NAMED(ctx, INTT_NAME[LM - 12], k_intt_contig<LM>, g, b, 0, data, col_stride, p.log_n, Winv, data2,
-                            gw);
     });
 }
 
@@ -309,47 +332,51 @@
                            uint32_t* out, uint64_t out_col_stride, uint32_t ncols, uint32_t beta0, uint32_t n_beta,
                            const uint32_t* scale, const uint32_t* evals2, const uint32_t* scale2, uint32_t gw,
                            uint32_t own_a, uint32_t own_b) {
-    const uint32_t *W = ctx.d_twiddle_fwd, *Winv = ctx.d_twiddle_inv;
+    const TwTables W = twiddles_fwd(ctx), Winv = twiddles_inv(ctx);
     const dim3 grid(p.tiles, ncols), b(NT_MID);
     const dim3 grid1(p.tiles * ncols);
 #define TS_MID_ARGS \
     evals, in_col_stride, out, out_col_stride, p.log_n, p.log_len, p.log_T, p.row_shift, beta0, n_beta, W, Winv, scale, \
         evals2, scale2, gw, own_a, own_b
+#define TS_MID_K(PLAN, TILE, LM, OWN) \
+    (k_lde_mid<PLAN, TILE, NT_MID, LM, OWN, typename MidForm<PLAN, TILE>::Fwd, typename MidForm<PLAN, TILE>::Inv>)
     if (own_a != LDE_NO_OWN && p.mid == NttMid::FIXED256 && p.LM == 12)
-        TS_LAUNCH_NAMED(ctx, "k_lde_mid<1>", (k_lde_mid<1, TILE_ELEMS, NT_MID, 12, true>), grid1, b, 0, TS_MID_ARGS);
+        TS_LAUNCH_NAMED(ctx, "k_lde_mid<1>", TS_MID_K(1, TILE_ELEMS, 12, true), grid1, b, 0, TS_MID_ARGS);
     else if (own_a != LDE_NO_OWN && p.mid == NttMid::FIXED256 && p.LM == 13)
-        TS_LAUNCH_NAMED(ctx, "(k_lde_mid<1, 8192, 512, 13>)", (k_lde_mid<1, 8192, 512, 13, true>), grid1, b, 0,
+        TS_LAUNCH_NAMED(ctx, "(k_lde_mid<1, 8192, 512, 13>)", TS_MID_K(1, 8192, 13, true), grid1, b, 0,
                         TS_MID_ARGS);
     else if (own_a != LDE_NO_OWN && p.mid == NttMid::FIXED256)
-        TS_LAUNCH_NAMED(ctx, "(k_lde_mid<1, 8192, 512, 14>)", (k_lde_mid<1, 8192, 512, 14, true>), grid1, b, 0,
+        TS_LAUNCH_NAMED(ctx, "(k_lde_mid<1, 8192, 512, 14>)", TS_MID_K(1, 8192, 14, true), grid1, b, 0,
                         TS_MID_ARGS);
     else if (own_a != LDE_NO_OWN)
-        TS_LAUNCH_NAMED(ctx, "k_lde_mid<0>", (k_lde_mid<0, TILE_ELEMS, NT_MID, LOG_M, true>), grid, b, 0, TS_MID_ARGS);
+        TS_LAUNCH_NAMED(ctx, "k_lde_mid<0>", TS_MID_K(0, TILE_ELEMS, LOG_M, true), grid, b, 0, TS_MID_ARGS);
     else if (p.mid == NttMid::TILE16384)
-        TS_LAUNCH_NAMED(ctx, "(k_lde_mid<0, 16384>)", (k_lde_mid<0, 16384>), grid, b, 0, TS_MID_ARGS);
+        TS_LAUNCH_NAMED(ctx, "(k_lde_mid<0, 16384>)", TS_MID_K(0, 16384, LOG_M, false), grid, b, 0, TS_MID_ARGS);
     else if (p.mid == NttMid::FIXED256 && p.LM == 12)
-        TS_LAUNCH_NAMED(ctx, "k_lde_mid<1>", k_lde_mid<1>, grid1, b, 0, TS_MID_ARGS);
+        TS_LAUNCH_NAMED(ctx, "k_lde_mid<1>", TS_MID_K(1, TILE_ELEMS, LOG_M, false), grid1, b, 0, TS_MID_ARGS);
     else if (p.mid == NttMid::FIXED256 && p.LM == 13)
-        TS_LAUNCH_NAMED(ctx, "(k_lde_mid<1, 8192, 512, 13>)", (k_lde_mid<1, 8192, 512, 13>), grid1, b, 0, TS_MID_ARGS);
+        TS_LAUNCH_NAMED(ctx, "(k_lde_mid<1, 8192, 512, 13>)", TS_MID_K(1, 8192, 13, false), grid1, b, 0, TS_MID_ARGS);
     else if (p.mid == NttMid::FIXED256)
-        TS_LAUNCH_NAMED(ctx, "(k_lde_mid<1, 8192, 512, 14>)", (k_lde_mid<1, 8192, 512, 14>), grid1, b, 0, TS_MID_ARGS);
+        TS_LAUNCH_NAMED(ctx, "(k_lde_mid<1, 8192, 512, 14>)", TS_MID_K(1, 8192, 14, false), grid1, b, 0, TS_MID_ARGS);
     else
-        TS_LAUNCH_NAMED(ctx, "k_lde_mid<0>", k_lde_mid<0>, grid, b, 0, TS_MID_ARGS);
+        TS_LAUNCH_NAMED(ctx, "k_lde_mid<0>", TS_MID_K(0, TILE_ELEMS, LOG_M, false), grid, b, 0, TS_MID_ARGS);
 #undef TS_MID_ARGS
+#undef TS_MID_K
 }
 
 void launch_contig_forward(Context& ctx, const NttPlan& p, uint32_t* data, uint64_t col_stride, uint32_t ncols,
                            uint32_t n_blocks, uint32_t gw, uint32_t own_a, uint32_t own_b) {
-    const uint32_t* W = ctx.d_twiddle_fwd;
+    const TwTables W = twiddles_fwd(ctx);
     with_chunk_log(p.LM, [&](auto lm) {
         constexpr int LM = decltype(lm)::value;
+        using TW = typename ContigForm<LM>::Fwd;
         constexpr int CPW = LM == 14 ? 4 : 1;
         if (own_a != LDE_NO_OWN)
-            TS_LAUNCH_NAMED(ctx, FWD_NAME[LM - 12], (k_lde_fwd_contig_own<LM, CPW>),
+            TS_LAUNCH_NAMED(ctx, FWD_NAME[LM - 12], (k_lde_fwd_contig_own<LM, CPW, TW>),
                             dim3(p.chunks / CPW, ncols, n_blocks - 1), dim3(chunk_threads(LM)), 0, data, col_stride,
                             p.log_n, W, gw, own_a, own_b);
         else
-            TS_LAUNCH_NAMED(ctx, FWD_NAME[LM - 12], (k_lde_fwd_contig<LM, CPW>), dim3(p.chunks / CPW, ncols, n_blocks),
+            TS_LAUNCH_NAMED(ctx, FWD_NAME[LM - 12], (k_lde_fwd_contig<LM, CPW, TW>), dim3(p.chunks / CPW, ncols, n_blocks),
                             dim3(chunk_threads(LM)), 0, data, col_stride, p.log_n, W);
     });
 }
@@ -374,6 +401,7 @@
     TS_REQUIRE(!first_round_done || p.fused_first_round, TS_ERR_INVARIANT,
                "coset_lde: no contiguous inverse pass at this size");
     ctx.ensure_twiddles(log_n == 0 ? 1 : log_n);
+    ctx.ensure_plant_twiddles(log_n == 0 ? 1 : log_n);
 
     const uint32_t n_cosets = 1u << log_blowup;
     if (n_beta == 0) n_beta = n_cosets - beta0;
diff --git a/tap-stark_amd/csrc/ntt_rounds.hpp b/tap-stark_amd/csrc/ntt_rounds.hpp
--- a/tap-stark_amd/csrc/ntt_rounds.hpp
+++ b/tap-stark_amd/csrc/ntt_rounds.hpp
@@ -10,23 +10,45 @@
 __device__ __forceinline__ uint32_t pad(uint32_t i) { return i + (i >> 5); }
 constexpr int padded(int n) { return n + (n >> 5); }
 
-template <int K, bool INV, bool TOP>
+template <class TW> struct TwForm;
+template <> struct TwForm<uint32_t> {
+    static constexpr bool plantard = false;
+    static __device__ __forceinline__ uint32_t mul(uint32_t a, uint32_t w) { return mont_mul(a, w); }
+    static __device__ __forceinline__ uint32_t mul_lazy(uint32_t a, uint32_t w) { return mont_mul_lazy(a, w); }
+};
+template <> struct TwForm<uint2> {
+    static constexpr bool plantard = true;
+    static __device__ __forceinline__ uint32_t mul(uint32_t a, uint2 w) { return plant_mul(a, w.x, w.y); }
+    static __device__ __forceinline__ uint32_t mul_lazy(uint32_t a, uint2 w) { return mul(a, w); }
+};
+
+struct TwTables {
+    const uint32_t* mont;
+    const uint2* plant;
+    operator const uint32_t*() const { return mont; }
+    operator const uint2*() const { return plant; }
+};
+inline TwTables twiddles_fwd(const Context& ctx) { return TwTables{ctx.d_twiddle_fwd, ctx.d_plant_fwd}; }
+inline TwTables twiddles_inv(const Context& ctx) { return TwTables{ctx.d_twiddle_inv, ctx.d_plant_inv}; }
+
+template <int K, bool INV, bool TOP, class TW>
 __device__ __forceinline__ void radix_butterflies(uint32_t (&v)[1 << K], unsigned s_base, unsigned u0,
                                                   uint32_t c, uint32_t hi,
-                                                  const uint32_t* __restrict__ W) {
+                                                  const TW* __restrict__ W) {
+    using F = TwForm<TW>;
     constexpr int R = 1 << K;
     if (!INV) {
 #pragma unroll
         for (int d = 0; d < K; d++) {
             const int half = R >> (d + 1);
-            const uint32_t* __restrict__ wp = W + ((1u << (s_base + u0 + d)) + (c << (u0 + d)) + (hi << d));
+            const TW* __restrict__ wp = W + ((1u << (s_base + u0 + d)) + (c << (u0 + d)) + (hi << d));
 #pragma unroll
             for (int q = 0; q < R; q++) {
                 if ((q & half) == 0) {
                     const uint32_t a = red2p(v[q]);
                     uint32_t t = v[q + half];
                     if (TOP && (q >> (K - d)) == 0) t = red2p(t);
-                    else t = mont_mul(t, wp[q >> (K - d)]);
+                    else t = F::mul(t, wp[q >> (K - d)]);
                     v[q] = a + t;
                     v[q + half] = a - t + P;
                 }
@@ -36,25 +58,32 @@
 #pragma unroll
         for (int d = K - 1; d >= 0; d--) {
             const int half = R >> (d + 1);
-            const uint32_t* __restrict__ wp = W + ((1u << (s_base + u0 + d)) + (c << (u0 + d)) + (hi << d));
+            const TW* __restrict__ wp = W + ((1u << (s_base + u0 + d)) + (c << (u0 + d)) + (hi << d));
 #pragma unroll
             for (int q = 0; q < R; q++) {
                 if ((q & half) == 0) {
-                    const uint32_t a = red2p(v[q]), b = red2p(v[q + half]);
-                    v[q] = a + b;
-                    uint32_t dlt = a - b + P;
-                    if (!(TOP && (q >> (K - d)) == 0)) dlt = mont_mul_lazy(dlt, wp[q >> (K - d)]);
-                    v[q + half] = dlt;
+                    const bool one = TOP && (q >> (K - d)) == 0;
+                    if (F::plantard) {
+                        const uint32_t a = v[q], b = v[q + half];
+                        v[q] = add(a, b);
+                        v[q + half] = one ? sub(a, b) : F::mul(a - b + P, wp[q >> (K - d)]);
+                    } else {
+                        const uint32_t a = red2p(v[q]), b = red2p(v[q + half]);
+                        v[q] = a + b;
+                        uint32_t dlt = a - b + P;
+                        if (!one) dlt = F::mul_lazy(dlt, wp[q >> (K - d)]);
+                        v[q + half] = dlt;
+                    }
                 }
             }
         }
     }
 }
 
-template <int K, bool INV, int LOG_DL, int NTH, bool TOP = false>
+template <int K, bool INV, int LOG_DL, int NTH, bool TOP = false, class TW>
 __device__ __forceinline__ void radix_round(uint32_t* s, unsigned log_total, unsigned u0,
                                             unsigned s_base, uint32_t c,
-                                            const uint32_t* __restrict__ W) {
+                                            const TW* __restrict__ W) {
     constexpr int R = 1 << K;
     const unsigned log_dl = LOG_DL >= 0 ? (unsigned)LOG_DL : log_total - u0 - K;
     const uint32_t n_groups = 1u << (log_total - K);
@@ -92,10 +121,10 @@
     __syncthreads();
 }
 
-template <bool INV, int NTH>
+template <bool INV, int NTH, class TW>
 __device__ __forceinline__ void radix_round_rt(int k, uint32_t* s, unsigned log_total, unsigned u0,
                                                unsigned s_base, uint32_t c,
-                                               const uint32_t* __restrict__ W) {
+                                               const TW* __restrict__ W) {
     switch (k) {
         case 4: radix_round<4, INV, -1, NTH>(s, log_total, u0, s_base, c, W); break;
         case 3: radix_round<3, INV, -1, NTH>(s, log_total, u0, s_base, c, W); break;
@@ -104,10 +133,10 @@
     }
 }
 
-template <int NTH>
+template <int NTH, class TW>
 __device__ __forceinline__ void tile_forward_rt(uint32_t* s, unsigned log_len, unsigned log_T,
                                                 unsigned s_base, uint32_t c,
-                                                const uint32_t* __restrict__ W) {
+                                                const TW* __restrict__ W) {
     if (log_len == 0) return;
     const unsigned nr = (log_len + 3) / 4, q = log_len / nr, rem = log_len % nr;
     unsigned u = 0;
@@ -117,10 +146,10 @@
         u += k;
     }
 }
-template <int NTH>
+template <int NTH, class TW>
 __device__ __forceinline__ void tile_inverse_rt(uint32_t* s, unsigned log_len, unsigned log_T,
                                                 unsigned s_base, uint32_t c,
-                                                const uint32_t* __restrict__ Winv) {
+                                                const TW* __restrict__ Winv) {
     if (log_len == 0) return;
     const unsigned nr = (log_len + 3) / 4, q = log_len / nr, rem = log_len % nr;
     unsigned u = log_len;
@@ -164,8 +193,8 @@
     }
 }
 
-template <int LM, bool INV, bool SKIP_R16 = false>
-__device__ __forceinline__ void chunk_rounds(uint32_t* s, unsigned sb, uint32_t c, const uint32_t* __restrict__ W) {
+template <int LM, bool INV, bool SKIP_R16 = false, class TW>
+__device__ __forceinline__ void chunk_rounds(uint32_t* s, unsigned sb, uint32_t c, const TW* __restrict__ W) {
     constexpr int NT = chunk_threads(LM);
     constexpr int K0 = LM == 12 ? 4 : 5;
     constexpr int K1 = LM == 14 ? 5 : 4;
diff --git a/tap-stark_amd/probe/field_probe.hip b/tap-stark_amd/probe/field_probe.hip
--- a/tap-stark_amd/probe/field_probe.hip
+++ b/tap-stark_amd/probe/field_probe.hip
@@ -42,7 +42,15 @@
     N_SCALAR_OPS = 26,
     OP_BFLY = 32,
     OP_BFLY_END = 36,
+    OP_PLANT_CONSTS = 40,
+    OP_PLANT_CONST = 41,
+    OP_PLANT_MUL = 42,
+    OP_PLANT_BFLY = 48,
+    OP_PLANT_BFLY_END = 52,
 };
+constexpr bool device_only(uint32_t op) {
+    return (op >= OP_BFLY && op < OP_BFLY_END) || (op >= OP_PLANT_BFLY && op < OP_PLANT_BFLY_END);
+}
 
 struct Shape {
     uint32_t n_in, n_out;
@@ -61,7 +69,12 @@
         case OP_EF_INV_PARTS: return {4, 5};
         case OP_EF_POW: return {6, 4};
         case OP_POW_CANON: case OP_MONT_POW: return {3, 1};
-        default: return (op >= OP_BFLY && op < OP_BFLY_END) ? Shape{32, 16} : Shape{0, 0};
+        case OP_PLANT_CONSTS: case OP_PLANT_CONST: return {1, 2};
+        case OP_PLANT_MUL: return {2, 1};
+        default:
+            return (op >= OP_BFLY && op < OP_BFLY_END)               ? Shape{32, 16}
+                   : (op >= OP_PLANT_BFLY && op < OP_PLANT_BFLY_END) ? Shape{48, 16}
+                                                                     : Shape{0, 0};
     }
 }
 
@@ -120,6 +133,14 @@
         case OP_TWO_ADIC_GEN: out[0] = two_adic_generator(in[0]); break;
         case OP_POW_CANON: out[0] = pow_canon(in[0], u64_at(in + 1)); break;
         case OP_MONT_POW: out[0] = mont_pow(in[0], u64_at(in + 1)); break;
+        case OP_PLANT_CONSTS: out[0] = (uint32_t)P_INV64; out[1] = (uint32_t)(P_INV64 >> 32); break;
+        case OP_PLANT_CONST: {
+            const uint64_t w = plant_const(in[0]);
+            out[0] = (uint32_t)w;
+            out[1] = (uint32_t)(w >> 32);
+            break;
+        }
+        case OP_PLANT_MUL: out[0] = plant_mul(in[0], plant_const(in[1])); break;
         default: break;
     }
 }
@@ -139,6 +160,17 @@
     uint32_t v[16];
     for (int q = 0; q < 16; q++) v[q] = in[(size_t)i * 32 + q];
     radix_butterflies<4, INV, TOP>(v, 0, 0, 0, 0, in + (size_t)i * 32 + 16);
+    for (int q = 0; q < 16; q++) out[(size_t)i * 16 + q] = v[q];
+}
+
+template <bool INV, bool TOP>
+__global__ void __launch_bounds__(256) k_probe_plant_bfly(const uint32_t* __restrict__ in, uint32_t* __restrict__ out,
+                                                          uint32_t count) {
+    const uint32_t i = blockIdx.x * 256u + threadIdx.x;
+    if (i >= count) return;
+    uint32_t v[16];
+    for (int q = 0; q < 16; q++) v[q] = in[(size_t)i * 48 + q];
+    radix_butterflies<4, INV, TOP>(v, 0, 0, 0, 0, reinterpret_cast<const uint2*>(in + (size_t)i * 48 + 16));
     for (int q = 0; q < 16; q++) out[(size_t)i * 16 + q] = v[q];
 }
 
@@ -180,6 +212,10 @@
         case OP_BFLY + 1: k_probe_bfly<true, false><<<grid, block>>>(d_in, d_out, count); break;
         case OP_BFLY + 2: k_probe_bfly<false, true><<<grid, block>>>(d_in, d_out, count); break;
         case OP_BFLY + 3: k_probe_bfly<true, true><<<grid, block>>>(d_in, d_out, count); break;
+        case OP_PLANT_BFLY + 0: k_probe_plant_bfly<false, false><<<grid, block>>>(d_in, d_out, count); break;
+        case OP_PLANT_BFLY + 1: k_probe_plant_bfly<true, false><<<grid, block>>>(d_in, d_out, count); break;
+        case OP_PLANT_BFLY + 2: k_probe_plant_bfly<false, true><<<grid, block>>>(d_in, d_out, count); break;
+        case OP_PLANT_BFLY + 3: k_probe_plant_bfly<true, true><<<grid, block>>>(d_in, d_out, count); break;
         default: k_probe<<<grid, block>>>(op, d_in, d_out, count, sh.n_in, sh.n_out); break;
     }
     HIP_OR_FAIL(hipGetLastError());
@@ -233,7 +269,7 @@
                     in[pos + 2], in[pos + 3]);
             return 2;
         }
-        if (host && op >= N_SCALAR_OPS) {
+        if (host && device_only(op)) {
             fprintf(stderr, "field_probe: record %u: op %u exists in the device build only\n", r, op);
             return 2;
         }
```

Result: faster. 26.24 billion, median of 6 (+3.0%).
